# Keyteer/Mixed-precision_LU_Factorization

Measured on AMD Instinct MI355X. Metric: LU GFLOP/s at N=32768 (1/2/4/8 GPUs); IR iterations to ||r||/||b||<1e-12, higher is better.
Workload: dtype f64

## Files before the change

### include/mpf_c.h

```cpp
#ifndef MPF_C_H
#define MPF_C_H
#include <stdint.h>
#ifdef __cplusplus
extern "C" {
#endif

typedef struct mpf_ctx mpf_ctx;

enum { MPF_TRAIL_FP64 = 0, MPF_TRAIL_FP16 = 1, MPF_TRAIL_FP16X3 = 2 };

typedef struct mpf_opts {
    int32_t trailing;
    int32_t verbose;
    int32_t fused_panel;
    int32_t sync_timing;
    int32_t no_lookahead;
    int32_t superpanel;
    int32_t pivot_path;
    int32_t pivot_search;
} mpf_opts;

typedef struct mpf_stats {
    double ms_total;
    double ms_h2d, ms_d2h;
    double ms_hpanel, ms_laswp, ms_dpanel, ms_trsm, ms_gemm;
    int64_t n;
    int32_t nb, panels;
    int32_t hpanel_timeouts;
    int32_t info;
    int32_t gemm_launches;
    int32_t lookahead;
    int32_t superpanel;
    int32_t pivot_path;
    double gemm_flops;
    double gemm_bytes;
    double ms_gemm_big, gemm_big_flops, gemm_big_bytes;
    double ms_cvt;
    double ms_blockrow;
    int32_t gemm_big_launches;
    int32_t host_rows_streamed;
    int32_t host_late_segments;
    int32_t pivot_search;
} mpf_stats;

int mpf_create(mpf_ctx **out, int device);
int mpf_destroy(mpf_ctx *ctx);
int mpf_set_stream(mpf_ctx *ctx, void *hip_stream);
int mpf_synchronize(mpf_ctx *ctx);
const char *mpf_last_error(mpf_ctx *ctx);
int mpf_get_stats(mpf_ctx *ctx, mpf_stats *out);
int64_t mpf_hgetf2_capacity_rows(mpf_ctx *ctx, int32_t waiters, int32_t form);
int mpf_set_option(mpf_ctx *ctx, const char *name, int64_t value);
int mpf_get_option(mpf_ctx *ctx, const char *name, int64_t *value);
int mpf_option_name(int32_t index, char *buf, int64_t buflen);
int mpf_device_report(char *buf, int64_t buflen);


int mpf_factor_host(mpf_ctx *ctx, double *A_host, int64_t N, int32_t nb, int32_t *ipiv_host,
                    const mpf_opts *opts);
int mpf_trim(mpf_ctx *ctx);
int mpf_factor_dev(mpf_ctx *ctx, double *d_A, int64_t lda, int64_t N, int32_t nb, int32_t *d_ipiv,
                   const mpf_opts *opts);

int mpf_double_to_fp16(mpf_ctx *ctx, const double *d_in, uint16_t *d_out, int64_t n);
int mpf_hdiv(mpf_ctx *ctx, const uint16_t *d_a, const uint16_t *d_b, uint16_t *d_q, int64_t n);
int mpf_hgetf2_pivots(mpf_ctx *ctx, const double *d_A, int64_t lda, int32_t rows, int32_t cols,
                      int32_t ipiv_offset, int32_t *d_ipiv, uint16_t *d_panel16_out);
int mpf_hgetf2(mpf_ctx *ctx, uint16_t *d_panel16, int64_t ld, int32_t rows, int32_t cols,
               int32_t *d_ipiv_panel);
int mpf_laswp(mpf_ctx *ctx, double *d_A, int64_t lda, int64_t ncols, int32_t k, int32_t cols,
              const int32_t *d_ipiv_global);
int mpf_dgetf2_npv(mpf_ctx *ctx, double *d_P, int64_t ld, int32_t rows, int32_t cols, int32_t fused);
int mpf_dgetf2_piv(mpf_ctx *ctx, double *d_P, int64_t ld, int32_t rows, int32_t cols, int32_t fused,
                   int32_t ipiv_offset, int32_t *d_ipiv, int32_t *info );
int mpf_dgetf2_tp(mpf_ctx *ctx, double *d_P, int64_t ld, int32_t rows, int32_t cols, int32_t fused,
                  int32_t ipiv_offset, int32_t *d_ipiv, int32_t *info );
int mpf_dtrsm_llnu(mpf_ctx *ctx, int32_t m, int64_t n, const double *d_L, int64_t ldl, double *d_B,
                   int64_t ldb);
int mpf_dgemm_minus(mpf_ctx *ctx, int64_t m, int64_t n, int32_t k, const double *d_A, int64_t lda,
                    const double *d_B, int64_t ldb, double *d_C, int64_t ldc);

int mpf_hgemm_minus(mpf_ctx *ctx, int64_t m, int64_t n, int32_t k, const double *d_A, int64_t lda,
                    const double *d_B, int64_t ldb, double *d_C, int64_t ldc, int32_t split );

int mpf_hgemm_minus_f32(mpf_ctx *ctx, int64_t m, int64_t n, int32_t k, const double *d_A, int64_t lda,
                        const double *d_B, int64_t ldb, float *d_C, int64_t ldc, int32_t split);

int mpf_w32_from_f64(mpf_ctx *ctx, const double *d_A, int64_t lda, float *d_W, int64_t ldw, int64_t rows, int64_t cols);
int mpf_w32_to_f64(mpf_ctx *ctx, const float *d_W, int64_t ldw, double *d_A, int64_t lda, int64_t rows, int64_t cols);
int mpf_w32_laswp(mpf_ctx *ctx, float *d_W, int64_t ldw, int64_t ncols, int32_t k, int32_t cols, const int32_t *d_ipiv_global);

int mpf_matgen_dev(mpf_ctx *ctx, double *d_A, int64_t lda, int64_t N, int64_t skip);
int mpf_matgen_cols_dev(mpf_ctx *ctx, double *d_A, int64_t lda, int64_t N, int64_t skip, int64_t col0, int64_t ncols);
int mpf_matgen_state(int64_t call, uint32_t *out31);

int mpf_check_plu_dev(mpf_ctx *ctx, const double *d_A, int64_t lda, const double *d_LU, int64_t ldlu, const int32_t *d_ipiv,
                      int64_t N, double *max_abs_err, double *fro_rel_err);
int mpf_check_plu_host(const double *A, const double *LU, const int32_t *ipiv, int64_t N, double *max_abs_err, double *fro_rel_err);

typedef struct mpf_ir_stats {
    int32_t iterations;
    int32_t converged;
    double rel_residual;
    double history[32];
    double ms_total;
    int32_t stalled;
    int32_t reserved;
} mpf_ir_stats;
int mpf_solve_ir(mpf_ctx *ctx, const double *d_A, int64_t lda, const double *d_LU, int64_t ldlu,
                 const int32_t *d_ipiv, int64_t N, const double *d_b, double *d_x, int32_t max_iter,
                 double tol, mpf_ir_stats *stats);

int mpf_solve_ir_nrhs(mpf_ctx *ctx, const double *d_A, int64_t lda, const double *d_LU, int64_t ldlu, const int32_t *d_ipiv,
                      int64_t N, int32_t nrhs, const double *d_B, int64_t ldb, double *d_X, int64_t ldx, int32_t max_iter,
                      double tol, mpf_ir_stats *stats);

typedef struct mpf_gmres_stats {
    int32_t outer_iterations, inner_iterations, converged;
    int32_t budget_expired;
    double rel_residual;
    double history[32];
    double ms_total;
} mpf_gmres_stats;
int mpf_solve_gmres_ir(mpf_ctx *ctx, const double *d_A, int64_t lda, const double *d_LU, int64_t ldlu, const int32_t *d_ipiv,
                       int64_t N, const double *d_b, double *d_x, int32_t max_outer, int32_t restart, double tol,
                       mpf_gmres_stats *stats);

typedef struct mpf_gesv_stats {
    int32_t path;
    int32_t info;
    double ms_factor_fp16, ms_ir_fp16, ms_factor_fp64, ms_ir_fp64, ms_total;
    mpf_ir_stats ir_fp16, ir_final;
    double gmres_budget_ms;
    int32_t gmres_budget_expired, reserved;
} mpf_gesv_stats;
int mpf_gesv(mpf_ctx *ctx, const double *d_A, int64_t lda, int64_t N, int32_t nb, double *d_work, int32_t *d_ipiv,
             const double *d_b, double *d_x, int32_t max_iter, double tol,
             int32_t try_fp16 ,
             mpf_gesv_stats *stats);


int mpf_solve_ir_trans(mpf_ctx *ctx, const double *d_A, int64_t lda, const double *d_LU, int64_t ldlu, const int32_t *d_ipiv,
                       int64_t N, int32_t nrhs, const double *d_B, int64_t ldb, double *d_X, int64_t ldx, int32_t max_iter,
                       double tol, mpf_ir_stats *stats);

int mpf_lange(mpf_ctx *ctx, const double *d_A, int64_t lda, int64_t M, int64_t N, char norm, double *out);

int mpf_geequ(mpf_ctx *ctx, const double *d_A, int64_t lda, int64_t N, double *d_r, double *d_c, double *rowcnd, double *colcnd,
              double *amax);

typedef struct mpf_gecon_stats {
    int32_t solves;
    int32_t solves_t;
    int32_t iterations;
    int32_t reserved;
    double ainvnm;
    double ms_total;
} mpf_gecon_stats;
int mpf_gecon(mpf_ctx *ctx, const double *d_LU, int64_t ldlu, int64_t N, char norm, double anorm, double *rcond,
              mpf_gecon_stats *stats);

typedef struct mpf_gesvx_stats {
    int32_t path;
    int32_t info;
    int32_t equed;
    int32_t skipped_by_rcond;
    double rowcnd, colcnd, amax;
    double anorm;
    double kappa_max;
    double rcond_lowp;
    double rcond;
    double ms_equilibrate, ms_factor, ms_gecon, ms_ir, ms_total;
    mpf_ir_stats ir_lowp, ir_final;
} mpf_gesvx_stats;
int mpf_gesvx(mpf_ctx *ctx, const double *d_A, int64_t lda, int64_t N, int32_t nb, double *d_work, int32_t *d_ipiv,
              const double *d_b, double *d_x, int32_t trans, int32_t equilibrate, int32_t try_fp16, double kappa_max,
              int32_t max_iter, double tol, double *d_r, double *d_c, mpf_gesvx_stats *stats);


int mpf_getrs(mpf_ctx *ctx, int32_t trans, const double *d_LU, int64_t ldlu, const int32_t *d_ipiv, int64_t N,
              int32_t nrhs, double *d_B, int64_t ldb);

int mpf_solve_ir_block(mpf_ctx *ctx, int32_t trans, const double *d_A, int64_t lda, const double *d_LU, int64_t ldlu,
                       const int32_t *d_ipiv, int64_t N, int32_t nrhs, const double *d_B, int64_t ldb, double *d_X,
                       int64_t ldx, int32_t max_iter, double tol, mpf_ir_stats *stats);

int mpf_solve_gmres_ir_block(mpf_ctx *ctx, int32_t trans, const double *d_A, int64_t lda, const double *d_LU, int64_t ldlu,
                             const int32_t *d_ipiv, int64_t N, int32_t nrhs, const double *d_B, int64_t ldb, double *d_X, int64_t ldx,
                             int32_t max_outer, int32_t restart, double tol, mpf_gmres_stats *stats );

typedef struct mpf_gerfs_stats {
    int32_t iterations;
    int32_t lacn2_iterations;
    int32_t solves;
    int32_t reserved;
    double ms_total;
} mpf_gerfs_stats;
int mpf_gerfs(mpf_ctx *ctx, int32_t trans, const double *d_A, int64_t lda, const double *d_LU, int64_t ldlu,
              const int32_t *d_ipiv, int64_t N, int32_t nrhs, const double *d_B, int64_t ldb, double *d_X, int64_t ldx,
              int32_t itmax, double *ferr, double *berr, mpf_gerfs_stats *stats);

int mpf_gesvx_block(mpf_ctx *ctx, const double *d_A, int64_t lda, int64_t N, int32_t nb, double *d_work, int32_t *d_ipiv,
                    int32_t nrhs, const double *d_B, int64_t ldb, double *d_X, int64_t ldx,
                    int32_t trans, int32_t equilibrate, int32_t try_fp16, double kappa_max, int32_t max_iter, double tol,
                    int32_t itmax, double *d_r, double *d_c,
                    double *ferr, double *berr,
                    mpf_gesvx_stats *stats,
                    mpf_ir_stats *ir, mpf_gerfs_stats *rfs  );

typedef int (*mpf_bcast_fn)(void *user, void *d_buf, int64_t bytes, int32_t root, void *hip_stream);
typedef int (*mpf_allreduce_fn)(void *user, double *d_buf, int64_t count, void *hip_stream);
typedef struct mpf_dist {
    int32_t rank, world;
    mpf_bcast_fn bcast;
    mpf_allreduce_fn allreduce;
    void *user;
} mpf_dist;
int mpf_rccl_unique_id(void *out128);
int mpf_rccl_init(mpf_ctx *ctx, const void *id128, int32_t rank, int32_t world);
int mpf_rccl_destroy(mpf_ctx *ctx);
int mpf_rccl_version(void);
typedef struct mpf_rccl_info_t {
    int32_t version, has_comm, comm_count, comm_rank, has_p2p, device, visible_devices, reserved;
    int64_t bcast_calls, bcast_bytes, allreduce_calls, p2p_calls, p2p_bytes;
    int32_t link_type[16], link_hops[16], peer_access[16];
} mpf_rccl_info_t;
int mpf_rccl_info(mpf_ctx *ctx, mpf_rccl_info_t *out);
int mpf_rccl_bcast_probe(mpf_ctx *ctx, int64_t bytes, int32_t root, int32_t reps, double *ms_per_bcast);
int mpf_rccl_selftest(mpf_ctx *ctx);
int mpf_factor_dist(mpf_ctx *ctx, double *d_Aloc, int64_t ldloc, int64_t N, int32_t nb, int32_t *d_ipiv, const mpf_dist *dist,
                    const mpf_opts *opts);
typedef int (*mpf_p2p_fn)(void *user, void *d_buf, int64_t bytes, int32_t peer, int32_t send, void *hip_stream);
int mpf_dist_set_p2p(mpf_ctx *ctx, mpf_p2p_fn fn, void *user);
// ... 9 lines not shown
```

### mixed-precision_lu_factorization_amd/__init__.py

```python
import ctypes as C
import os
import subprocess

_HERE = os.path.dirname(os.path.abspath(__file__))
LIB_PATH = os.environ.get("MPF_LIB") or os.path.join(_HERE, "lib", "libmpf_amd.so")
PROBE_LIB_PATH = os.environ.get("MPF_PROBE_LIB") or os.path.join(_HERE, "lib", "libmpf_probe.so")

TRAIL_FP64 = 0
TRAIL_FP16 = 1
TRAIL_FP16X3 = 2

C_ABI_SYMBOLS = [
    "mpf_create", "mpf_destroy", "mpf_set_stream", "mpf_synchronize", "mpf_last_error", "mpf_get_stats",
    "mpf_device_report", "mpf_factor_host", "mpf_factor_dev", "mpf_double_to_fp16", "mpf_hdiv",
    "mpf_hgetf2_pivots", "mpf_hgetf2", "mpf_laswp", "mpf_dgetf2_npv", "mpf_dtrsm_llnu", "mpf_dgemm_minus",
    "mpf_solve_ir", "mpf_hgetf2_capacity_rows", "mpf_set_option", "mpf_get_option", "mpf_option_name", "mpf_hgemm_minus", "mpf_hgemm_minus_f32", "mpf_w32_from_f64", "mpf_w32_to_f64", "mpf_w32_laswp", "mpf_gesv", "mpf_matgen_dev", "mpf_matgen_cols_dev",
    "mpf_matgen_state", "mpf_rccl_unique_id", "mpf_rccl_init", "mpf_rccl_destroy", "mpf_rccl_version", "mpf_rccl_info", "mpf_rccl_bcast_probe", "mpf_factor_dist",
    "mpf_solve_ir_dist", "mpf_rccl_selftest", "mpf_check_plu_dev", "mpf_check_plu_host", "mpf_solve_ir_nrhs",
    "mpf_solve_gmres_ir", "mpf_trim", "mpf_dist_set_p2p",
    "mpf_solve_ir_trans", "mpf_lange", "mpf_geequ", "mpf_gecon", "mpf_gesvx",
    "mpf_getrs", "mpf_solve_ir_block", "mpf_gerfs", "mpf_gesvx_block",
    "mpf_dgetf2_piv", "mpf_solve_gmres_ir_block", "mpf_dgetf2_tp",
]
PROBE_ONLY_SYMBOLS = ["mpf_microbench", "mpf_debug_mfma4", "mpf_debug_gate", "mpf_debug_hgemm_again"]
CXX_SYMBOL_MPF = "_Z3MPFPdiiPi"


class MpfOpts(C.Structure):
    _fields_ = [("trailing", C.c_int32), ("verbose", C.c_int32), ("fused_panel", C.c_int32),
                ("sync_timing", C.c_int32), ("no_lookahead", C.c_int32), ("superpanel", C.c_int32), ("pivot_path", C.c_int32), ("pivot_search", C.c_int32)]


class MpfStats(C.Structure):
    _fields_ = [("ms_total", C.c_double), ("ms_h2d", C.c_double), ("ms_d2h", C.c_double),
                ("ms_hpanel", C.c_double), ("ms_laswp", C.c_double), ("ms_dpanel", C.c_double),
                ("ms_trsm", C.c_double), ("ms_gemm", C.c_double), ("n", C.c_int64), ("nb", C.c_int32),
                ("panels", C.c_int32), ("hpanel_timeouts", C.c_int32), ("info", C.c_int32),
                ("gemm_launches", C.c_int32), ("lookahead", C.c_int32), ("superpanel", C.c_int32),
                ("pivot_path", C.c_int32), ("gemm_flops", C.c_double), ("gemm_bytes", C.c_double),
                ("ms_gemm_big", C.c_double), ("gemm_big_flops", C.c_double), ("gemm_big_bytes", C.c_double),
                ("ms_cvt", C.c_double), ("ms_blockrow", C.c_double), ("gemm_big_launches", C.c_int32), ("host_rows_streamed", C.c_int32),
                ("host_late_segments", C.c_int32), ("pivot_search", C.c_int32)]


class MpfIrStats(C.Structure):
    _fields_ = [("iterations", C.c_int32), ("converged", C.c_int32), ("rel_residual", C.c_double),
                ("history", C.c_double * 32), ("ms_total", C.c_double), ("stalled", C.c_int32), ("reserved", C.c_int32)]


class MpfGmresStats(C.Structure):
    _fields_ = [("outer_iterations", C.c_int32), ("inner_iterations", C.c_int32), ("converged", C.c_int32), ("budget_expired", C.c_int32),
                ("rel_residual", C.c_double), ("history", C.c_double * 32), ("ms_total", C.c_double)]


class MpfRcclInfo(C.Structure):
    _fields_ = [("version", C.c_int32), ("has_comm", C.c_int32), ("comm_count", C.c_int32), ("comm_rank", C.c_int32), ("has_p2p", C.c_int32),
                ("device", C.c_int32), ("visible_devices", C.c_int32), ("reserved", C.c_int32),
                ("bcast_calls", C.c_int64), ("bcast_bytes", C.c_int64), ("allreduce_calls", C.c_int64), ("p2p_calls", C.c_int64), ("p2p_bytes", C.c_int64),
                ("link_type", C.c_int32 * 16), ("link_hops", C.c_int32 * 16), ("peer_access", C.c_int32 * 16)]


class MpfGesvStats(C.Structure):
    _fields_ = [("path", C.c_int32), ("info", C.c_int32), ("ms_factor_fp16", C.c_double), ("ms_ir_fp16", C.c_double),
                ("ms_factor_fp64", C.c_double), ("ms_ir_fp64", C.c_double), ("ms_total", C.c_double),
                ("ir_fp16", MpfIrStats), ("ir_final", MpfIrStats), ("gmres_budget_ms", C.c_double), ("gmres_budget_expired", C.c_int32),
                ("reserved", C.c_int32)]


class MpfGeconStats(C.Structure):
    _fields_ = [("solves", C.c_int32), ("solves_t", C.c_int32), ("iterations", C.c_int32), ("reserved", C.c_int32),
                ("ainvnm", C.c_double), ("ms_total", C.c_double)]


class MpfGesvxStats(C.Structure):
    _fields_ = [("path", C.c_int32), ("info", C.c_int32), ("equed", C.c_int32), ("skipped_by_rcond", C.c_int32),
                ("rowcnd", C.c_double), ("colcnd", C.c_double), ("amax", C.c_double), ("anorm", C.c_double), ("kappa_max", C.c_double),
                ("rcond_lowp", C.c_double), ("rcond", C.c_double), ("ms_equilibrate", C.c_double), ("ms_factor", C.c_double),
                ("ms_gecon", C.c_double), ("ms_ir", C.c_double), ("ms_total", C.c_double), ("ir_lowp", MpfIrStats), ("ir_final", MpfIrStats)]


class MpfGerfsStats(C.Structure):
    _fields_ = [("iterations", C.c_int32), ("lacn2_iterations", C.c_int32), ("solves", C.c_int32), ("reserved", C.c_int32),
                ("ms_total", C.c_double)]


BCAST_FN = C.CFUNCTYPE(C.c_int, C.c_void_p, C.c_void_p, C.c_int64, C.c_int32, C.c_void_p)
ALLREDUCE_FN = C.CFUNCTYPE(C.c_int, C.c_void_p, C.c_void_p, C.c_int64, C.c_void_p)
P2P_FN = C.CFUNCTYPE(C.c_int, C.c_void_p, C.c_void_p, C.c_int64, C.c_int32, C.c_int32, C.c_void_p)


class MpfDist(C.Structure):
    _fields_ = [("rank", C.c_int32), ("world", C.c_int32), ("bcast", BCAST_FN), ("allreduce", ALLREDUCE_FN), ("user", C.c_void_p)]


class MPFError(RuntimeError):
    pass


def build(force=False):
    srcs = [os.path.join(_HERE, "csrc", f) for f in os.listdir(os.path.join(_HERE, "csrc"))]
    srcs += [os.path.join(_HERE, "..", "include", h) for h in ("mpf_c.h", "MPF.h", "mpf_probe.h")] + [os.path.join(_HERE, "Makefile")]
    stale = force or any(not os.path.exists(lp) or any(os.path.getmtime(s) > os.path.getmtime(lp) for s in srcs)
                         for lp in (LIB_PATH, PROBE_LIB_PATH))
    if stale:
        subprocess.run(["make", "-C", _HERE, "-s", "-j8", "all", "probe"], check=True)
    return LIB_PATH


_libs = {}


def load_library(probe=False):
    if probe in _libs:
        return _libs[probe]
    import torch
    path = PROBE_LIB_PATH if probe else LIB_PATH
    if not os.path.exists(path):
        raise MPFError(f"{path} is missing: run `python -c 'import __graft_entry__ as g; g.build()'` "
                       "(there is no CPU fallback)")
    L = C.CDLL(path)
    vp, i32, i64, dbl = C.c_void_p, C.c_int32, C.c_int64, C.c_double
    L.mpf_create.argtypes = [C.POINTER(vp), C.c_int]
    L.mpf_destroy.argtypes = [vp]
    L.mpf_set_stream.argtypes = [vp, vp]
    L.mpf_synchronize.argtypes = [vp]
    L.mpf_last_error.argtypes = [vp]
    L.mpf_last_error.restype = C.c_char_p
    L.mpf_get_stats.argtypes = [vp, C.POINTER(MpfStats)]
    L.mpf_set_option.argtypes = [vp, C.c_char_p, i64]
    L.mpf_get_option.argtypes = [vp, C.c_char_p, C.POINTER(i64)]
    L.mpf_option_name.argtypes = [i32, C.c_char_p, i64]
    L.mpf_device_report.argtypes = [C.c_char_p, i64]
    L.mpf_factor_host.argtypes = [vp, vp, i64, i32, vp, C.POINTER(MpfOpts)]
    L.mpf_trim.argtypes = [vp]
    L.mpf_dist_set_p2p.argtypes = [vp, P2P_FN, vp]
    L.mpf_factor_dev.argtypes = [vp, vp, i64, i64, i32, vp, C.POINTER(MpfOpts)]
    L.mpf_double_to_fp16.argtypes = [vp, vp, vp, i64]
    L.mpf_hdiv.argtypes = [vp, vp, vp, vp, i64]
    L.mpf_hgetf2_pivots.argtypes = [vp, vp, i64, i32, i32, i32, vp, vp]
    L.mpf_hgetf2.argtypes = [vp, vp, i64, i32, i32, vp]
    L.mpf_laswp.argtypes = [vp, vp, i64, i64, i32, i32, vp]
    L.mpf_dgetf2_npv.argtypes = [vp, vp, i64, i32, i32, i32]
    L.mpf_dgetf2_piv.argtypes = [vp, vp, i64, i32, i32, i32, i32, vp, C.POINTER(i32)]
    L.mpf_dgetf2_tp.argtypes = [vp, vp, i64, i32, i32, i32, i32, vp, C.POINTER(i32)]
    L.mpf_dtrsm_llnu.argtypes = [vp, i32, i64, vp, i64, vp, i64]
    L.mpf_dgemm_minus.argtypes = [vp, i64, i64, i32, vp, i64, vp, i64, vp, i64]
    L.mpf_hgemm_minus.argtypes = [vp, i64, i64, i32, vp, i64, vp, i64, vp, i64, i32]
    L.mpf_hgemm_minus_f32.argtypes = [vp, i64, i64, i32, vp, i64, vp, i64, vp, i64, i32]
    L.mpf_w32_from_f64.argtypes = [vp, vp, i64, vp, i64, i64, i64]
    L.mpf_w32_to_f64.argtypes = [vp, vp, i64, vp, i64, i64, i64]
    L.mpf_w32_laswp.argtypes = [vp, vp, i64, i64, i32, i32, vp]
    L.mpf_solve_ir.argtypes = [vp, vp, i64, vp, i64, vp, i64, vp, vp, i32, dbl, C.POINTER(MpfIrStats)]
    L.mpf_solve_ir_nrhs.argtypes = [vp, vp, i64, vp, i64, vp, i64, i32, vp, i64, vp, i64, i32, dbl, C.POINTER(MpfIrStats)]
    L.mpf_solve_gmres_ir.argtypes = [vp, vp, i64, vp, i64, vp, i64, vp, vp, i32, i32, dbl, C.POINTER(MpfGmresStats)]
    L.mpf_gesv.argtypes = [vp, vp, i64, i64, i32, vp, vp, vp, vp, i32, dbl, i32, C.POINTER(MpfGesvStats)]
    L.mpf_solve_ir_trans.argtypes = [vp, vp, i64, vp, i64, vp, i64, i32, vp, i64, vp, i64, i32, dbl, C.POINTER(MpfIrStats)]
    L.mpf_lange.argtypes = [vp, vp, i64, i64, i64, C.c_char, C.POINTER(dbl)]
    L.mpf_geequ.argtypes = [vp, vp, i64, i64, vp, vp, C.POINTER(dbl), C.POINTER(dbl), C.POINTER(dbl)]
    L.mpf_gecon.argtypes = [vp, vp, i64, i64, C.c_char, dbl, C.POINTER(dbl), C.POINTER(MpfGeconStats)]
    L.mpf_gesvx.argtypes = [vp, vp, i64, i64, i32, vp, vp, vp, vp, i32, i32, i32, dbl, i32, dbl, vp, vp, C.POINTER(MpfGesvxStats)]
    L.mpf_getrs.argtypes = [vp, i32, vp, i64, vp, i64, i32, vp, i64]
    L.mpf_solve_ir_block.argtypes = [vp, i32, vp, i64, vp, i64, vp, i64, i32, vp, i64, vp, i64, i32, dbl, C.POINTER(MpfIrStats)]
    L.mpf_solve_gmres_ir_block.argtypes = [vp, i32, vp, i64, vp, i64, vp, i64, i32, vp, i64, vp, i64, i32, i32, dbl, C.POINTER(MpfGmresStats)]
    L.mpf_gerfs.argtypes = [vp, i32, vp, i64, vp, i64, vp, i64, i32, vp, i64, vp, i64, i32, C.POINTER(dbl), C.POINTER(dbl),
                            C.POINTER(MpfGerfsStats)]
    L.mpf_gesvx_block.argtypes = [vp, vp, i64, i64, i32, vp, vp, i32, vp, i64, vp, i64, i32, i32, i32, dbl, i32, dbl, i32, vp, vp,
                                  C.POINTER(dbl), C.POINTER(dbl), C.POINTER(MpfGesvxStats), C.POINTER(MpfIrStats), C.POINTER(MpfGerfsStats)]
    L.mpf_matgen_dev.argtypes = [vp, vp, i64, i64, i64]
    L.mpf_matgen_cols_dev.argtypes = [vp, vp, i64, i64, i64, i64, i64]
    L.mpf_matgen_state.argtypes = [i64, C.POINTER(C.c_uint32)]
    L.mpf_rccl_unique_id.argtypes = [vp]
    L.mpf_rccl_init.argtypes = [vp, vp, i32, i32]
    L.mpf_rccl_destroy.argtypes = [vp]
    L.mpf_rccl_version.argtypes = []
    L.mpf_rccl_selftest.argtypes = [vp]
    L.mpf_check_plu_dev.argtypes = [vp, vp, i64, vp, i64, vp, i64, C.POINTER(dbl), C.POINTER(dbl)]
    L.mpf_check_plu_host.argtypes = [vp, vp, vp, i64, C.POINTER(dbl), C.POINTER(dbl)]
    L.mpf_factor_dist.argtypes = [vp, vp, i64, i64, i32, vp, C.POINTER(MpfDist), C.POINTER(MpfOpts)]
    L.mpf_solve_ir_dist.argtypes = [vp, vp, i64, vp, i64, vp, i64, i32, vp, vp, i32, dbl, C.POINTER(MpfDist), C.POINTER(MpfIrStats)]
    for name in C_ABI_SYMBOLS:
        if name != "mpf_last_error":
            getattr(L, name).restype = C.c_int
    if probe:
        L.mpf_microbench.argtypes = [vp, C.c_int, C.POINTER(C.c_double)]
        L.mpf_microbench.restype = C.c_int
    _libs[probe] = L
    return L


def option_names():
    L = load_library()
    buf = C.create_string_buffer(64)
    n = L.mpf_option_name(-1, buf, 64)
    out = []
    for i in range(n):
        L.mpf_option_name(i, buf, 64)
        out.append(buf.value.decode())
    return out


def device_report():
    L = load_library()
    buf = C.create_string_buffer(4096)
    n = L.mpf_device_report(buf, 4096)
    return n, buf.value.decode()


def _ptr(t):
    return C.c_void_p(t.data_ptr()) if t is not None else C.c_void_p(0)


def _colmajor_ld(t):
    assert t.dim() == 2 and t.stride(0) == 1, "need a column-major matrix (e.g. X.t() of a contiguous tensor)"
    return t.stride(1) if t.shape[1] > 1 else max(t.shape[0], 1)


class MPFContext:

    def __init__(self, device=0, use_torch_stream=True, stream=None, probe=False, options=None):
        import torch
        if not torch.cuda.is_available():
            raise MPFError("no GPU visible: the MPF hot path is HIP-only (no CPU fallback)")
        self.torch = torch
        self.probe = probe
        self.L = load_library(probe)
        self.h = C.c_void_p()
        rc = self.L.mpf_create(C.byref(self.h), device)
        if rc != 0:
            raise MPFError("mpf_create failed: " + self.L.mpf_last_error(None).decode())
        self.device = torch.device("cuda", device)
        self.stream = stream
        self._follow = stream is None and use_torch_stream
        self._bound = None
        if stream is not None:
            self.L.mpf_set_stream(self.h, C.c_void_p(stream.cuda_stream))
        self._bind()
        for k, v in (options or {}).items():
            self.set_option(k, v)

    def set_option(self, name, value):
        self._check(self.L.mpf_set_option(self.h, name.encode(), int(value)), "mpf_set_option")

    def rccl_info(self):
        inf = MpfRcclInfo()
        self.L.mpf_rccl_info.argtypes = [C.c_void_p, C.POINTER(MpfRcclInfo)]
        self._check(self.L.mpf_rccl_info(self.h, C.byref(inf)), "mpf_rccl_info")
        nd = min(int(inf.visible_devices), 16)
        return {"version": int(inf.version), "has_comm": bool(inf.has_comm), "comm_count": int(inf.comm_count), "comm_rank": int(inf.comm_rank),
                "has_p2p": bool(inf.has_p2p), "device": int(inf.device), "visible_devices": int(inf.visible_devices),
                "bcast_calls": int(inf.bcast_calls), "bcast_bytes": int(inf.bcast_bytes), "allreduce_calls": int(inf.allreduce_calls),
                "p2p_calls": int(inf.p2p_calls), "p2p_bytes": int(inf.p2p_bytes),
                "link_type_to_device": [int(inf.link_type[d]) for d in range(nd)], "link_hops_to_device": [int(inf.link_hops[d]) for d in range(nd)],
                "peer_access_to_device": [int(inf.peer_access[d]) for d in range(nd)]}

    def rccl_bcast_probe(self, nbytes, root=0, reps=5):
        self._bind()
        ms = C.c_double(0)
        self.L.mpf_rccl_bcast_probe.argtypes = [C.c_void_p, C.c_int64, C.c_int32, C.c_int32, C.POINTER(C.c_double)]
        self._check(self.L.mpf_rccl_bcast_probe(self.h, int(nbytes), int(root), int(reps), C.byref(ms)), "mpf_rccl_bcast_probe")
        return ms.value

    def hgetf2_capacity_rows(self, waiters=0, form=0):
        self.L.mpf_hgetf2_capacity_rows.argtypes = [C.c_void_p, C.c_int32, C.c_int32]
        self.L.mpf_hgetf2_capacity_rows.restype = C.c_int64
        return int(self.L.mpf_hgetf2_capacity_rows(self.h, waiters, form))

    def get_option(self, name):
        v = C.c_int64(0)
        self._check(self.L.mpf_get_option(self.h, name.encode(), C.byref(v)), "mpf_get_option")
        return v.value

    def _bind(self):
        if self._follow:
            cur = self.torch.cuda.current_stream(self.device).cuda_stream
            if cur != self._bound:
                self.L.mpf_set_stream(self.h, C.c_void_p(cur))
                self._bound = cur

    def close(self):
        if self.h:
            self.L.mpf_destroy(self.h)
            self.h = C.c_void_p()

    def __del__(self):
        try:
            self.close()
        except Exception:
            pass

    def _check(self, rc, what):
        if rc < 0:
            raise MPFError(f"{what} failed ({rc}): " + self.L.mpf_last_error(self.h).decode())
        return rc

    def colmajor(self, rows, cols, dtype=None):
        t = self.torch
        return t.empty((cols, rows), dtype=dtype or t.float64, device=self.device).t()

    def from_numpy_f(self, a):
# ... 79 lines not shown
        n, nrhs = B.shape
        X = self.colmajor(n, nrhs)
        st = (MpfIrStats * nrhs)()
        rc = self.L.mpf_solve_ir_nrhs(self.h, _ptr(A), _colmajor_ld(A), _ptr(LU), _colmajor_ld(LU), _ptr(ipiv), n, nrhs,
                                      _ptr(B), _colmajor_ld(B), _ptr(X), _colmajor_ld(X), max_iter, tol, st)
        self._check(rc, "mpf_solve_ir_nrhs")
        return X, list(st)

    def solve_gmres_ir(self, A, LU, ipiv, b, max_outer=10, restart=30, tol=1e-12):
        self._bind()
        t = self.torch
        n = A.shape[0]
        x = t.empty(n, dtype=t.float64, device=self.device)
        st = MpfGmresStats()
        rc = self.L.mpf_solve_gmres_ir(self.h, _ptr(A), _colmajor_ld(A), _ptr(LU), _colmajor_ld(LU), _ptr(ipiv), n, _ptr(b), _ptr(x),
                                       max_outer, restart, tol, C.byref(st))
        self._check(rc, "mpf_solve_gmres_ir")
        return x, st

    def check_plu(self, A, LU, ipiv):
        self._bind()
        mx, fro = C.c_double(0), C.c_double(0)
        rc = self.L.mpf_check_plu_dev(self.h, _ptr(A), _colmajor_ld(A), _ptr(LU), _colmajor_ld(LU), _ptr(ipiv), A.shape[0],
                                      C.byref(mx), C.byref(fro))
        self._check(rc, "mpf_check_plu_dev")
        return mx.value, fro.value

    def rccl_init(self, rank, world, group=None):
        import torch.distributed as tdist
        ident = [None]
        if world == 1:
            buf = C.create_string_buffer(128)
            self._check(self.L.mpf_rccl_unique_id(buf), "mpf_rccl_unique_id")
            self._check(self.L.mpf_rccl_init(self.h, buf, 0, 1), "mpf_rccl_init")
            return
        loaded = [int(self.L.mpf_rccl_version() > 0)]
        everyone = [None] * world
        tdist.all_gather_object(everyone, loaded[0], group=group)
        if not all(everyone):
            raise RuntimeError(f"librccl not loadable on ranks {[r for r, ok in enumerate(everyone) if not ok]}")
        if rank == 0:
            buf = C.create_string_buffer(128)
            if self.L.mpf_rccl_unique_id(buf) == 0:
                ident[0] = bytes(buf.raw)
        tdist.broadcast_object_list(ident, src=0, group=group)
        if ident[0] is None:
            raise RuntimeError("mpf_rccl_unique_id failed on rank 0 (librccl not loadable?)")
        self._check(self.L.mpf_rccl_init(self.h, C.c_char_p(ident[0]), rank, world), "mpf_rccl_init")

    def dist_set_p2p(self, fn):
        self._bind()
        self._check(self.L.mpf_dist_set_p2p(self.h, fn if fn is not None else C.cast(None, P2P_FN), None), "mpf_dist_set_p2p")

    def factor_dist(self, Aloc, n, nb, dist, ipiv=None, trailing=TRAIL_FP64, no_lookahead=False, pivot_path=0, verbose=False, superpanel=0,
                    pivot_search=0):
        self._bind()
        t = self.torch
        if ipiv is None:
            ipiv = t.arange(1, n + 1, dtype=t.int32, device=self.device)
        o = MpfOpts(trailing=trailing, no_lookahead=int(no_lookahead), pivot_path=int(pivot_path), verbose=int(verbose), superpanel=int(superpanel),
                    pivot_search=int(pivot_search))
        ld = _colmajor_ld(Aloc) if Aloc.shape[1] > 0 else n
        rc = self.L.mpf_factor_dist(self.h, _ptr(Aloc) if Aloc.shape[1] > 0 else C.c_void_p(0), max(ld, n), n, nb, _ptr(ipiv),
                                    C.byref(dist), C.byref(o))
        return ipiv, self._check(rc, "mpf_factor_dist")

    def solve_ir_dist(self, Aloc, LUloc, ipiv, b, n, nb, dist, max_iter=10, tol=1e-12):
        self._bind()
        t = self.torch
        x = t.empty(n, dtype=t.float64, device=self.device)
        st = MpfIrStats()
        has = Aloc.shape[1] > 0
        rc = self.L.mpf_solve_ir_dist(self.h, _ptr(Aloc) if has else C.c_void_p(0), max(_colmajor_ld(Aloc), n) if has else n,
                                      _ptr(LUloc) if has else C.c_void_p(0), max(_colmajor_ld(LUloc), n) if has else n, _ptr(ipiv),
                                      n, nb, _ptr(b), _ptr(x), max_iter, tol, C.byref(dist), C.byref(st))
        self._check(rc, "mpf_solve_ir_dist")
        return x, st

    def double_to_fp16(self, x):
        self._bind()
        t = self.torch
        out = t.empty(x.numel(), dtype=t.int16, device=self.device)
        self._check(self.L.mpf_double_to_fp16(self.h, _ptr(x), _ptr(out), x.numel()), "double_to_fp16")
        return out

    def hdiv(self, a_bits, b_bits):
        self._bind()
        t = self.torch
        q = t.empty_like(a_bits)
        self._check(self.L.mpf_hdiv(self.h, _ptr(a_bits), _ptr(b_bits), _ptr(q), a_bits.numel()), "hdiv")
        return q

    def hgetf2_pivots(self, P, ipiv_offset=0, want_panel=False):
        self._bind()
        t = self.torch
        rows, cols = P.shape
        ipiv = t.zeros(cols, dtype=t.int32, device=self.device)
        out = self.colmajor(rows, cols, dtype=t.int16) if want_panel else None
        rc = self.L.mpf_hgetf2_pivots(self.h, _ptr(P), _colmajor_ld(P), rows, cols, ipiv_offset, _ptr(ipiv), _ptr(out))
        self._check(rc, "hgetf2_pivots")
        return ipiv, out

    def hgetf2(self, P16):
        self._bind()
        t = self.torch
        rows, cols = P16.shape
        ipiv = t.zeros(cols, dtype=t.int32, device=self.device)
        self._check(self.L.mpf_hgetf2(self.h, _ptr(P16), _colmajor_ld(P16), rows, cols, _ptr(ipiv)), "hgetf2")
        return ipiv

    def laswp(self, A, k, cols, ipiv_global):
        self._bind()
        self._check(self.L.mpf_laswp(self.h, _ptr(A), _colmajor_ld(A), A.shape[1], k, cols, _ptr(ipiv_global)), "laswp")

    def dgetf2_npv(self, P, fused=False):
        self._bind()
        rows, cols = P.shape
        self._check(self.L.mpf_dgetf2_npv(self.h, _ptr(P), _colmajor_ld(P), rows, cols, int(fused)), "dgetf2_npv")

    def dgetf2_piv(self, P, fused=False, ipiv_offset=0):
        self._bind()
        t = self.torch
        rows, cols = P.shape
        ipiv = t.zeros(min(rows, cols), dtype=t.int32, device=self.device)
        info = C.c_int32(0)
        self._check(self.L.mpf_dgetf2_piv(self.h, _ptr(P), _colmajor_ld(P), rows, cols, int(fused), int(ipiv_offset), _ptr(ipiv),
                                          C.byref(info)), "dgetf2_piv")
        return ipiv, info.value

    def dgetf2_tp(self, P, fused=False, ipiv_offset=0):
        self._bind()
        t = self.torch
        rows, cols = P.shape
        ipiv = t.zeros(min(rows, cols), dtype=t.int32, device=self.device)
        info = C.c_int32(0)
        self._check(self.L.mpf_dgetf2_tp(self.h, _ptr(P), _colmajor_ld(P), rows, cols, int(fused), int(ipiv_offset), _ptr(ipiv),
                                         C.byref(info)), "dgetf2_tp")
        return ipiv, info.value

    def dtrsm_llnu(self, Lm, B):
        self._bind()
        m, n = B.shape
        assert Lm.shape[0] >= m and Lm.shape[1] >= m, "dtrsm_llnu: L smaller than m x m"
        self._check(self.L.mpf_dtrsm_llnu(self.h, m, n, _ptr(Lm), _colmajor_ld(Lm), _ptr(B), _colmajor_ld(B)), "dtrsm")

    def dgemm_minus(self, Cm, A, B):
        self._bind()
        m, n = Cm.shape
        k = A.shape[1]
        assert A.shape == (m, k) and B.shape == (k, n), "dgemm_minus: operand shapes do not match C"
        self._check(self.L.mpf_dgemm_minus(self.h, m, n, k, _ptr(A), _colmajor_ld(A), _ptr(B), _colmajor_ld(B),
                                           _ptr(Cm), _colmajor_ld(Cm)), "dgemm")

    def hgemm_minus(self, Cm, A, B, split=False):
        self._bind()
        m, n = Cm.shape
        k = A.shape[1]
        assert A.shape == (m, k) and B.shape == (k, n), "hgemm_minus: operand shapes do not match C"
        self._check(self.L.mpf_hgemm_minus(self.h, m, n, k, _ptr(A), _colmajor_ld(A), _ptr(B), _colmajor_ld(B),
                                           _ptr(Cm), _colmajor_ld(Cm), int(split)), "hgemm")

    def hgemm_minus_f32(self, Cm, A, B, split=False):
        self._bind()
        assert Cm.dtype == self.torch.float32
        m, n = Cm.shape
        k = A.shape[1]
        assert A.shape == (m, k) and B.shape == (k, n), "hgemm_minus_f32: operand shapes do not match C"
        self._check(self.L.mpf_hgemm_minus_f32(self.h, m, n, k, _ptr(A), _colmajor_ld(A), _ptr(B), _colmajor_ld(B),
                                               _ptr(Cm), _colmajor_ld(Cm), int(split)), "hgemm_f32")

    def w32_from_f64(self, A, W):
        self._bind()
        rows, cols = A.shape
        assert W.shape == (rows, cols) and W.dtype == self.torch.float32 and W.stride(1) == 1
        self._check(self.L.mpf_w32_from_f64(self.h, _ptr(A), _colmajor_ld(A), _ptr(W), W.stride(0), rows, cols), "w32_from_f64")

    def w32_to_f64(self, W, A):
        self._bind()
        rows, cols = A.shape
        assert W.shape == (rows, cols) and W.dtype == self.torch.float32 and W.stride(1) == 1
        self._check(self.L.mpf_w32_to_f64(self.h, _ptr(W), W.stride(0), _ptr(A), _colmajor_ld(A), rows, cols), "w32_to_f64")

    def w32_laswp(self, W, k, cols, ipiv_global):
        self._bind()
        assert W.dtype == self.torch.float32 and W.stride(1) == 1
        self._check(self.L.mpf_w32_laswp(self.h, _ptr(W), W.stride(0), W.shape[1], k, cols, _ptr(ipiv_global)), "w32_laswp")

    def gesv(self, A, b, nb=256, max_iter=10, tol=1e-12, try_fp16=True, work=None):
        self._bind()
        t = self.torch
        n = A.shape[0]
        if work is None:
            work = self.colmajor(n, n)
        ipiv = t.empty(n, dtype=t.int32, device=self.device)
        x = t.empty(n, dtype=t.float64, device=self.device)
        st = MpfGesvStats()
        rc = self.L.mpf_gesv(self.h, _ptr(A), _colmajor_ld(A), n, nb, _ptr(work), _ptr(ipiv), _ptr(b), _ptr(x), max_iter, tol,
                             int(try_fp16), C.byref(st))
        self._check(rc, "mpf_gesv")
        return x, st, work, ipiv

    def solve_ir_trans(self, A, LU, ipiv, B, max_iter=10, tol=1e-12):
        self._bind()
        n = A.shape[0]
        vec = B.dim() == 1
        nrhs = 1 if vec else B.shape[1]
        X = self.torch.empty(n, dtype=self.torch.float64, device=self.device) if vec else self.colmajor(n, nrhs)
        st = (MpfIrStats * max(nrhs, 1))()
        ldb = n if vec else _colmajor_ld(B)
        ldx = n if vec else _colmajor_ld(X)
        rc = self.L.mpf_solve_ir_trans(self.h, _ptr(A), _colmajor_ld(A), _ptr(LU), _colmajor_ld(LU), _ptr(ipiv), n, nrhs,
                                       _ptr(B), ldb, _ptr(X), ldx, max_iter, tol, st)
        self._check(rc, "mpf_solve_ir_trans")
        return X, (st[0] if vec else list(st)[:nrhs])

    def lange(self, A, norm="1"):
        self._bind()
        m, n = A.shape
        out = C.c_double(0)
        ld = _colmajor_ld(A) if m > 0 and n > 0 else max(m, 1)
        self._check(self.L.mpf_lange(self.h, _ptr(A), ld, m, n, norm.encode()[:1], C.byref(out)), "mpf_lange")
        return out.value

    def geequ(self, A):
        self._bind()
        t = self.torch
        n = A.shape[0]
        r = t.zeros(n, dtype=t.float64, device=self.device)
        c = t.zeros(n, dtype=t.float64, device=self.device)
        rc_, cc_, am = C.c_double(0), C.c_double(0), C.c_double(0)
        info = self._check(self.L.mpf_geequ(self.h, _ptr(A), _colmajor_ld(A), n, _ptr(r), _ptr(c), C.byref(rc_), C.byref(cc_), C.byref(am)),
                           "mpf_geequ")
        return r, c, rc_.value, cc_.value, am.value, info

    def gecon(self, LU, anorm, norm="1"):
        self._bind()
        rcond = C.c_double(0)
        st = MpfGeconStats()
        self._check(self.L.mpf_gecon(self.h, _ptr(LU), _colmajor_ld(LU), LU.shape[0], norm.encode()[:1], float(anorm), C.byref(rcond),
                                     C.byref(st)), "mpf_gecon")
        return rcond.value, st

    def cond(self, A, LU, ipiv=None, norm="1"):
        anorm = self.lange(A, norm)
        rcond, _ = self.gecon(LU, anorm, norm)
        return float("inf") if rcond == 0 else 1.0 / rcond

    def gesvx(self, A, b, nb=256, trans=False, equilibrate=1, try_fp16=1, kappa_max=0.0, max_iter=10, tol=1e-12, work=None,
              want_scales=False):
        self._bind()
        t = self.torch
        n = A.shape[0]
        if work is None:
            work = self.colmajor(n, n)
        ipiv = t.empty(n, dtype=t.int32, device=self.device)
        x = t.empty(n, dtype=t.float64, device=self.device)
        r = t.empty(n, dtype=t.float64, device=self.device) if want_scales else None
        c = t.empty(n, dtype=t.float64, device=self.device) if want_scales else None
        st = MpfGesvxStats()
        rc = self.L.mpf_gesvx(self.h, _ptr(A), _colmajor_ld(A), n, nb, _ptr(work), _ptr(ipiv), _ptr(b), _ptr(x), int(bool(trans)),
                              int(equilibrate), int(try_fp16), float(kappa_max), max_iter, tol, _ptr(r), _ptr(c), C.byref(st))
        self._check(rc, "mpf_gesvx")
        out = (x, st, work, ipiv)
        return out + (r, c) if want_scales else out

    def _rhs(self, B):
        if B.dim() == 1:
            return B.view(-1, 1), 1, max(B.shape[0], 1)
        return B, B.shape[1], _colmajor_ld(B)

    def getrs(self, LU, ipiv, B, trans=False, overwrite=False):
        self._bind()
        n = LU.shape[0]
        if overwrite:
            X = B
        elif B.dim() == 1:
            X = B.clone()
        else:
            X = self.colmajor(n, B.shape[1])
            X.copy_(B)
        _, nrhs, ldx = self._rhs(X)
        rc = self.L.mpf_getrs(self.h, int(bool(trans)), _ptr(LU), _colmajor_ld(LU), _ptr(ipiv), n, nrhs, _ptr(X), ldx)
        self._check(rc, "mpf_getrs")
        return X

    def solve_ir_block(self, A, LU, ipiv, B, trans=False, max_iter=10, tol=1e-12):
        self._bind()
        n = A.shape[0]
        vec = B.dim() == 1
        _, nrhs, ldb = self._rhs(B)
        X = self.torch.empty(n, dtype=self.torch.float64, device=self.device) if vec else self.colmajor(n, nrhs)
        ldx = n if vec else _colmajor_ld(X)
        st = (MpfIrStats * max(nrhs, 1))()
        rc = self.L.mpf_solve_ir_block(self.h, int(bool(trans)), _ptr(A), _colmajor_ld(A), _ptr(LU), _colmajor_ld(LU), _ptr(ipiv), n,
                                       nrhs, _ptr(B), ldb, _ptr(X), ldx, max_iter, tol, st)
        self._check(rc, "mpf_solve_ir_block")
        return X, list(st)[:nrhs]

    def solve_gmres_ir_block(self, A, LU, ipiv, B, trans=False, max_outer=10, restart=30, tol=1e-12):
        self._bind()
        n = A.shape[0]
        vec = B.dim() == 1
        _, nrhs, ldb = self._rhs(B)
        X = self.torch.empty(n, dtype=self.torch.float64, device=self.device) if vec else self.colmajor(n, nrhs)
        ldx = n if vec else _colmajor_ld(X)
        st = (MpfGmresStats * max(nrhs, 1))()
# ... 57 lines not shown
```

### mixed-precision_lu_factorization_amd/csrc/mpf_host.cpp

```cpp
#include "solve_common.h"
#include "../../include/MPF.h"
#include <climits>
#include <cstdio>
#include <cstdlib>
#include <cstring>
#include <cmath>
#include <iostream>
#include <vector>
#include <mutex>
#include <functional>
#include <chrono>

static thread_local std::string g_noctx_err;

namespace {
struct OptDesc { const char *name, *env; size_t off; bool wide; long long lo, hi; };
#define OPT_I(field, env, lo, hi) {#field, env, offsetof(MpfTuning, field), false, lo, hi}
#define OPT_L(field, env, lo, hi) {#field, env, offsetof(MpfTuning, field), true, lo, hi}
const OptDesc kOpts[] = {
    OPT_I(safe_pivots, "MPF_SAFE_PIVOTS", 0, 1),
    OPT_I(pivot_fp64, "MPF_PIVOT_FP64", 0, 2),
    OPT_I(chain_pipeline, "MPF_CHAIN_PIPELINE", 0, 1),
    OPT_L(chain_pipeline_below, "MPF_CHAIN_PIPELINE_BELOW", 0, 1ll << 40),
    OPT_I(fp16_work32, "MPF_FP16_WORK32", 0, 1),
    OPT_I(superpanel_fp16, "MPF_SUPERPANEL", 0, 8),
    OPT_I(superpanel_fp64, "MPF_SUPERPANEL_FP64", 1, 8),
    OPT_I(no_lookahead, "MPF_NO_LOOKAHEAD", 0, 1),
    OPT_I(verbose, "MPF_VERBOSE", 0, 1),
    OPT_I(timeline, "MPF_TIMELINE", 0, 1),
    OPT_L(hp_spin_limit, "MPF_HP_SPIN_LIMIT", 1, 1ll << 31),
    OPT_L(hp_gate_ticks, "MPF_HP_GATE_TICKS", 0, 1ll << 40),
    OPT_I(hp_acq_fence, "MPF_HP_ACQ_FENCE", 0, 1),
    OPT_I(hp_window, "MPF_HP_WINDOW", -1, 1 << 30),
    OPT_I(hgemm_pad, "MPF_HGEMM_PAD", 0, 65536),
    OPT_I(hgemm_split_pad, "MPF_HGEMM_SPLIT_PAD", 0, 65536),
    OPT_I(hgemm_big, "MPF_HGEMM_BIG", 0, 1),
    OPT_I(hgemm_big_tile, "MPF_HGEMM_BIG_TILE", 0, 5),
    OPT_I(hgemm_mfma16, "MPF_HGEMM_MFMA16", 0, 1),
    OPT_I(dgemm_dma, "MPF_DGEMM_DMA", 0, 1),
    OPT_I(lazy_gather, "MPF_LAZY_GATHER", 0, 1),
    OPT_I(dpanel_fused_form, "MPF_DPANEL_FUSED", 0, 1),
    OPT_I(dist_instalments, "MPF_DIST_INSTALMENTS", 0, 1),
    OPT_L(dist_instalment_min_bytes, "MPF_DIST_INSTALMENT_MIN_BYTES", 0, 1ll << 40),
    OPT_I(generic_fused, "MPF_GENERIC_FUSED", 0, 1),
    OPT_I(fp64_rowmajor, "MPF_FP64_ROWMAJOR", 0, 1),
    OPT_L(fp64_rowmajor_min_n, "MPF_FP64_ROWMAJOR_MIN_N", 0, 1ll << 40),
    OPT_I(trsm_laswp_fused, "MPF_TRSM_LASWP_FUSED", 0, 1),
    OPT_I(fp64_two_lanes, "MPF_FP64_TWO_LANES", 0, 1 << 30),
    OPT_I(fp64_lane_a_pct, "MPF_FP64_LANE_A_PCT", 20, 90),
    OPT_I(fp64_pair, "MPF_FP64_PAIR", 0, 1),
    OPT_L(fp64_pair_min_n, "MPF_FP64_PAIR_MIN_N", 0, 1ll << 40),
    OPT_I(event_timers, "MPF_EVENT_TIMERS", 0, 2),
    OPT_I(dist_world1_loop, "MPF_DIST_WORLD1_LOOP", 0, 1),
    OPT_I(gesv_fp64_tflops, "MPF_GESV_FP64_TFLOPS", 0, 1000),
    OPT_I(gate_wait_value, "MPF_GATE_WAIT_VALUE", 0, 1),
    OPT_I(host_sink, "MPF_HOST_SINK", 0, 1),
    OPT_I(sink_trace, "MPF_SINK_TRACE", 0, 1),
    OPT_I(hp_half_slabs, "MPF_HP_HALF_SLABS", 0, 1),
    OPT_I(hp_half_slabs_rows, "MPF_HP_HALF_SLABS_ROWS", 256, 32768),
    OPT_I(hp_local_xcd, "MPF_HP_LOCAL_XCD", 0, 2),
    OPT_I(host_late_parts, "MPF_HOST_LATE_PARTS", 0, 4),
    OPT_L(host_late_min_n, "MPF_HOST_LATE_MIN_N", 0, 1ll << 40),
    OPT_I(host_first_pct, "MPF_HOST_FIRST_PCT", 5, 100),
    OPT_I(host_late_q_pct, "MPF_HOST_LATE_Q_PCT", 1, 1000),
    OPT_L(host_sink_min_n, "MPF_HOST_SINK_MIN_N", 0, 1ll << 40),
    OPT_I(dist_solve_p2p, "MPF_DIST_SOLVE_P2P", 0, 1),
    OPT_I(gmres_group_tiles, "MPF_GMRES_GROUP_TILES", 0, 16),
#ifdef MPF_PROBE
    OPT_I(hp_stamp, "MPF_HP_STAMP", 0, 1),
    OPT_I(hp_r256_upto, "MPF_HP_R256_UPTO", 0, 1 << 30),
    OPT_I(dgemm_w8, "MPF_DGEMM_W8", 0, 1),
    OPT_I(gemm_lds_pad, "MPF_GEMM_LDS_PAD", 0, 65536),
    OPT_I(hgemm_big_reg, "MPF_HGEMM_BIG_REG", 0, 1),
    OPT_I(hgemm_dbg, "MPF_HGEMM_DBG", 0, 8191),
#endif
};
#undef OPT_I
#undef OPT_L
void opt_store(MpfTuning &t, const OptDesc &d, long long v) {
    if (v < d.lo) v = d.lo;
    if (v > d.hi) v = d.hi;
    char *p = (char *)&t + d.off;
    if (d.wide) *(long long *)p = v; else *(int *)p = (int)v;
}
long long opt_load(const MpfTuning &t, const OptDesc &d) {
    const char *p = (const char *)&t + d.off;
    return d.wide ? *(const long long *)p : (long long)*(const int *)p;
}
void tuning_from_env(MpfTuning &t) {
    for (const OptDesc &d : kOpts)
        if (const char *e = getenv(d.env)) if (*e) opt_store(t, d, atoll(e));
}
}

static int fail(mpf_ctx *c, int code, const std::string &msg) {
    if (c) c->err = msg; else g_noctx_err = msg;
    return code;
}

extern "C" {

int mpf_create(mpf_ctx **out, int device) {
    if (!out) return -1;
    *out = nullptr;
    int ndev = 0;
    hipError_t e = hipGetDeviceCount(&ndev);
    if (e != hipSuccess || ndev == 0) return fail(nullptr, -3, "No HIP devices available.");
    if (device < 0 || device >= ndev) return fail(nullptr, -1, "mpf_create: bad device index");
    mpf_ctx *c = new mpf_ctx();
    tuning_from_env(c->tune);
    c->device = device;
    if (hipSetDevice(device) != hipSuccess) { delete c; return fail(nullptr, -2, "hipSetDevice failed"); }
    hipDeviceProp_t prop;
    if (hipGetDeviceProperties(&prop, device) == hipSuccess) c->num_cus = prop.multiProcessorCount;
    if (hipStreamCreateWithFlags(&c->stream, hipStreamNonBlocking) != hipSuccess) { delete c; return fail(nullptr, -2, "hipStreamCreate failed"); }
    c->own_stream = true;
    {
        int lo = 0, hi = 0;
        hipDeviceGetStreamPriorityRange(&lo, &hi);
        if (hipStreamCreateWithPriority(&c->pstream, hipStreamNonBlocking, hi) != hipSuccess) c->pstream = nullptr;
        if (hipStreamCreateWithPriority(&c->tstream, hipStreamNonBlocking, hi) != hipSuccess) c->tstream = nullptr;
    }
    if (hipMalloc((void **)&c->ws, sizeof(MpfWorkspace)) != hipSuccess) { hipStreamDestroy(c->stream); delete c; return fail(nullptr, -2, "hipMalloc(workspace) failed"); }
    hipMemset(c->ws, 0, sizeof(MpfWorkspace));
    if (hipExtMallocWithFlags((void **)&c->hp_signal, 8, hipMallocSignalMemory) != hipSuccess) { c->hp_signal = nullptr; (void)hipGetLastError(); }
    else hipMemset(c->hp_signal, 0, 8);
    hipEventCreate(&c->ev0);
    hipEventCreate(&c->ev1);
    *out = c;
    return 0;
}

int mpf_destroy(mpf_ctx *c) {
    if (!c) return 0;
    hipSetDevice(c->device);
    if (c->stream) hipStreamSynchronize(c->stream);
    if (c->ws) hipFree(c->ws);
    if (c->hp_signal) hipFree(c->hp_signal);
    mpf_rccl_destroy(c);
    sink_destroy(c);
    feed_destroy(c);
    if (c->ev0) hipEventDestroy(c->ev0);
    if (c->ev1) hipEventDestroy(c->ev1);
    if (c->pstream) { hipStreamSynchronize(c->pstream); hipStreamDestroy(c->pstream); }
    if (c->tstream) { hipStreamSynchronize(c->tstream); hipStreamDestroy(c->tstream); }
    if (c->xstream) { hipStreamSynchronize(c->xstream); hipStreamDestroy(c->xstream); }
    for (hipEvent_t e : c->ev_pool) hipEventDestroy(e);
    if (c->own_stream && c->stream) hipStreamDestroy(c->stream);
    delete c;
    return 0;
}

int mpf_set_stream(mpf_ctx *c, void *hip_stream) {
    if (!c) return -1;
    if (c->own_stream && c->stream) { hipStreamSynchronize(c->stream); hipStreamDestroy(c->stream); }
    c->stream = (hipStream_t)hip_stream;
    c->own_stream = false;
    return 0;
}

int mpf_synchronize(mpf_ctx *c) {
    if (!c) return -1;
    MPF_HIP_TRY(c, hipStreamSynchronize(c->stream));
    return 0;
}

const char *mpf_last_error(mpf_ctx *c) { return c ? c->err.c_str() : g_noctx_err.c_str(); }

int mpf_get_stats(mpf_ctx *c, mpf_stats *out) {
    if (!c || !out) return -1;
    *out = c->stats;
    return 0;
}

int mpf_set_option(mpf_ctx *c, const char *name, int64_t value) {
    if (!c || !name) return -1;
    for (const OptDesc &d : kOpts)
        if (!strcmp(d.name, name)) {
            opt_store(c->tune, d, (long long)value);
            c->attr_done = 0; c->attr_big = 0;
            return 0;
        }
    return fail(c, -1, std::string("mpf_set_option: unknown option '") + name + "'");
}
int mpf_get_option(mpf_ctx *c, const char *name, int64_t *value) {
    if (!c || !name || !value) return -1;
    for (const OptDesc &d : kOpts)
        if (!strcmp(d.name, name)) { *value = (int64_t)opt_load(c->tune, d); return 0; }
    return fail(c, -1, std::string("mpf_get_option: unknown option '") + name + "'");
}
int mpf_option_name(int32_t index, char *buf, int64_t buflen) {
    const int n = (int)(sizeof kOpts / sizeof kOpts[0]);
    if (index >= 0 && index < n && buf && buflen > 0) { strncpy(buf, kOpts[index].name, (size_t)buflen - 1); buf[buflen - 1] = 0; }
    return n;
}

int mpf_device_report(char *buf, int64_t buflen) {
    int ndev = 0;
    if (hipGetDeviceCount(&ndev) != hipSuccess) ndev = 0;
    std::string s = "HIP devices: " + std::to_string(ndev) + "\n";
    int rt = 0, drv = 0;
    if (ndev > 0 && hipRuntimeGetVersion(&rt) == hipSuccess && hipDriverGetVersion(&drv) == hipSuccess)
        s += "HIP runtime " + std::to_string(rt) + " driver " + std::to_string(drv) + "\n";
    const int rv = ndev > 0 ? mpf_rccl_version() : -1;
    s += rv > 0 ? "RCCL version " + std::to_string(rv / 10000) + "." + std::to_string(rv / 100 % 100) + "." + std::to_string(rv % 100) + " (NCCL API, dlopen)\n"
                : std::string("RCCL: not loaded\n");
    for (int d = 0; d < ndev; ++d) {
        hipDeviceProp_t p;
        if (hipGetDeviceProperties(&p, d) != hipSuccess) continue;
        int coop = 0, lds_cu = 0, l2 = 0, clk = 0, memclk = 0, buswidth = 0;
        hipDeviceGetAttribute(&coop, hipDeviceAttributeCooperativeLaunch, d);
        hipDeviceGetAttribute(&lds_cu, hipDeviceAttributeMaxSharedMemoryPerMultiprocessor, d);
        hipDeviceGetAttribute(&l2, hipDeviceAttributeL2CacheSize, d);
        hipDeviceGetAttribute(&clk, hipDeviceAttributeClockRate, d);
        hipDeviceGetAttribute(&memclk, hipDeviceAttributeMemoryClockRate, d);
        hipDeviceGetAttribute(&buswidth, hipDeviceAttributeMemoryBusWidth, d);
        char line[768];
        snprintf(line, sizeof line,
                 "device %d: %s arch %s CUs %d maxThreadsPerBlock %d LDS/block %zu B LDS/CU %d B warpSize %d regs/block %d "
                 "L2 %d KiB clock %d MHz memclock %d MHz bus %d bit HBM %.1f GiB cooperativeLaunch %d pivot-kernel rows/launch %d\n",
                 d, p.name, p.gcnArchName, p.multiProcessorCount, p.maxThreadsPerBlock, p.sharedMemPerBlock, lds_cu, p.warpSize,
                 p.regsPerBlock, l2 / 1024, clk / 1000, memclk / 1000, buswidth, (double)p.totalGlobalMem / (1024.0 * 1024.0 * 1024.0), coop,
                 HP_R * (p.multiProcessorCount < HP_MAXG ? p.multiProcessorCount : HP_MAXG));
        s += line;
    }
    if (ndev > 1) {
        s += "link matrix (type:hops, type 4 = xGMI; P = peer access):\n";
        for (int a = 0; a < ndev; ++a) {
            std::string row = "  dev " + std::to_string(a) + ":";
            for (int b = 0; b < ndev; ++b) {
                if (a == b) { row += "   -  "; continue; }
                uint32_t lt = 0, hops = 0;
                int peer = 0;
                hipDeviceCanAccessPeer(&peer, a, b);
                if (hipExtGetLinkTypeAndHopCount(a, b, &lt, &hops) != hipSuccess) { lt = 0; hops = 0; }
                char cell[32];
                snprintf(cell, sizeof cell, " %u:%u%s", lt, hops, peer ? "P" : " ");
                row += cell;
            }
            s += row + "\n";
        }
    }
    if (buf && buflen > 0) { strncpy(buf, s.c_str(), (size_t)buflen - 1); buf[buflen - 1] = 0; }
    return ndev;
}

int mpf_double_to_fp16(mpf_ctx *c, const double *d_in, uint16_t *d_out, int64_t n) {
    if (!c) return -1;
    return launch_double_to_fp16(c, d_in, d_out, n);
}
int mpf_hdiv(mpf_ctx *c, const uint16_t *a, const uint16_t *b, uint16_t *q, int64_t n) {
    if (!c) return -1;
    return launch_hdiv(c, a, b, q, n);
}
int mpf_hgetf2_pivots(mpf_ctx *c, const double *d_A, int64_t lda, int32_t rows, int32_t cols, int32_t ipiv_offset,
                      int32_t *d_ipiv, uint16_t *d_panel16_out) {
    if (!c || !d_A || !d_ipiv) return -1;
    if (lda < rows) return fail(c, -1, "hgetf2_pivots: lda < rows");
    if (cols > 65535) return fail(c, -1, "hgetf2_pivots: panel width > 65535");
    if (!safe_pivots(c) && hgetf2_lds_eligible(c, rows, cols))
        return launch_hgetf2(c, d_A, lda, nullptr, 0, rows, cols, ipiv_offset, d_ipiv, d_panel16_out, rows, nullptr);
    return launch_hgetf2_generic(c, d_A, lda, nullptr, 0, rows, cols, ipiv_offset, d_ipiv, d_panel16_out, rows);
}
int mpf_hgetf2(mpf_ctx *c, uint16_t *d_panel16, int64_t ld, int32_t rows, int32_t cols, int32_t *d_ipiv_panel) {
    if (!c || !d_panel16 || !d_ipiv_panel) return -1;
    if (ld < rows) return fail(c, -1, "hgetf2: ld < rows");
    if (!safe_pivots(c) && hgetf2_lds_eligible(c, rows, cols))
        return launch_hgetf2(c, nullptr, 0, d_panel16, ld, rows, cols, 0, d_ipiv_panel, nullptr, 0, nullptr);
    return launch_hgetf2_generic(c, nullptr, 0, d_panel16, ld, rows, cols, 0, d_ipiv_panel, nullptr, 0);
}
int mpf_laswp(mpf_ctx *c, double *d_A, int64_t lda, int64_t ncols, int32_t k, int32_t cols, const int32_t *d_ipiv) {
    if (!c || !d_A || !d_ipiv) return -1;
    if (cols > HP_MAXCOLS) return launch_laswp_seq(c, d_A, lda, ncols, k, cols, d_ipiv, lda);
    return launch_laswp(c, d_A, lda, ncols, k, cols, d_ipiv);
}
int mpf_dgetf2_npv(mpf_ctx *c, double *d_P, int64_t ld, int32_t rows, int32_t cols, int32_t fused) {
    if (!c || !d_P) return -1;
    if (ld < rows) return fail(c, -1, "dgetf2_npv: ld < rows");
    return launch_dgetf2_npv(c, d_P, ld, rows, cols, fused, 0);
}
int mpf_dgetf2_piv(mpf_ctx *c, double *d_P, int64_t ld, int32_t rows, int32_t cols, int32_t fused, int32_t ipiv_offset,
                   int32_t *d_ipiv, int32_t *info) {
    if (!c || !d_P || !d_ipiv) return -1;
    if (rows < 1 || cols < 1 || cols > 65535) return fail(c, -1, "dgetf2_piv: need rows >= 1 and 1 <= cols <= 65535");
    if (ld < rows) return fail(c, -1, "dgetf2_piv: ld < rows");
    MPF_HIP_TRY(c, hipSetDevice(c->device));
    const int imax = INT_MAX;
    MPF_HIP_TRY(c, hipMemcpyAsync(&c->ws->info, &imax, sizeof(int), hipMemcpyHostToDevice, c->stream));
    const int rc = launch_dgetf2_piv(c, d_P, ld, rows, cols, fused, 0, ipiv_offset, d_ipiv);
    if (rc || !info) return rc;
    int v = 0;
    MPF_HIP_TRY(c, hipMemcpyAsync(&v, &c->ws->info, sizeof(int), hipMemcpyDeviceToHost, c->stream));
    MPF_HIP_TRY(c, hipStreamSynchronize(c->stream));
    *info = v == INT_MAX ? 0 : v;
    return 0;
}
int mpf_dgetf2_tp(mpf_ctx *c, double *d_P, int64_t ld, int32_t rows, int32_t cols, int32_t fused, int32_t ipiv_offset,
                  int32_t *d_ipiv, int32_t *info) {
    if (!c || !d_P || !d_ipiv) return -1;
    if (rows < 1 || cols < 1 || cols > 65535) return fail(c, -1, "dgetf2_tp: need rows >= 1 and 1 <= cols <= 65535");
    if (ld < rows) return fail(c, -1, "dgetf2_tp: ld < rows");
    MPF_HIP_TRY(c, hipSetDevice(c->device));
    const int imax = INT_MAX;
    MPF_HIP_TRY(c, hipMemcpyAsync(&c->ws->info, &imax, sizeof(int), hipMemcpyHostToDevice, c->stream));
    const int rc = launch_dgetf2_tp(c, d_P, ld, rows, cols, fused, 0, ipiv_offset, d_ipiv);
    if (rc || !info) return rc;
    int v = 0;
    MPF_HIP_TRY(c, hipMemcpyAsync(&v, &c->ws->info, sizeof(int), hipMemcpyDeviceToHost, c->stream));
    MPF_HIP_TRY(c, hipStreamSynchronize(c->stream));
    *info = v == INT_MAX ? 0 : v;
    return 0;
}
int mpf_dtrsm_llnu(mpf_ctx *c, int32_t m, int64_t n, const double *d_L, int64_t ldl, double *d_B, int64_t ldb) {
    if (!c) return -1;
    if (m > 0 && n > 0 && (ldl < m || ldb < m)) return fail(c, -1, "dtrsm: leading dimension < m");
    return launch_dtrsm_llnu(c, m, n, d_L, ldl, d_B, ldb);
}
int mpf_dgemm_minus(mpf_ctx *c, int64_t m, int64_t n, int32_t k, const double *d_A, int64_t lda, const double *d_B,
                    int64_t ldb, double *d_C, int64_t ldc) {
    if (!c) return -1;
    if (m > 0 && n > 0 && k > 0 && (lda < m || ldb < k || ldc < m)) return fail(c, -1, "dgemm: bad leading dimension");
    return launch_dgemm_minus(c, m, n, k, d_A, lda, d_B, ldb, d_C, ldc);
}

int mpf_ensure_h_images(mpf_ctx *c, int64_t rows, int kmax, bool big) {
    kmax = (kmax + 63) & ~63;
    if (c->h_L && c->h_rows >= rows && c->h_kmax >= kmax && (!big || c->h_Lb[0])) return 0;
    if (rows < c->h_rows) rows = c->h_rows;
    if (kmax < c->h_kmax) kmax = c->h_kmax;
    big = big || c->h_Lb[0];
    c->h_L.release(); c->h_U.release();
    for (auto &b : c->h_Lb) b.release();
    c->h_rows = 0; c->h_kmax = 0;
    const int64_t elems = 2 * rows * kmax;
    MPF_HIP_TRY(c, c->h_L.grow(elems));
    MPF_HIP_TRY(c, c->h_U.grow(elems));
    if (big) for (auto &b : c->h_Lb) MPF_HIP_TRY(c, b.grow(elems));
    c->h_rows = rows; c->h_kmax = kmax;
    return 0;
}

int mpf_hgemm_minus(mpf_ctx *c, int64_t m, int64_t n, int32_t k, const double *d_A, int64_t lda, const double *d_B,
                    int64_t ldb, double *d_C, int64_t ldc, int32_t split) {
    if (!c) return -1;
    if (m <= 0 || n <= 0 || k <= 0) return 0;
    if (k > 8 * HP_MAXCOLS) return fail(c, -1, "hgemm: k > 2048");
    if (lda < m || ldb < k || ldc < m) return fail(c, -1, "hgemm: bad leading dimension");
    int rc = mpf_ensure_h_images(c, m > n ? m : n, k, false);
    if (!rc) rc = launch_cvt_l21(c, d_A, lda, m, k, split);
    if (!rc) rc = launch_hgemm_minus(c, m, n, k, d_B, ldb, d_C, ldc, split);
    return rc;
}

int mpf_hgemm_minus_f32(mpf_ctx *c, int64_t m, int64_t n, int32_t k, const double *d_A, int64_t lda, const double *d_B,
                        int64_t ldb, float *d_C, int64_t ldc, int32_t split) {
    if (!c || !d_A || !d_B || !d_C) return -1;
    if (m <= 0 || n <= 0 || k <= 0) return 0;
    if (k > 8 * HP_MAXCOLS) return fail(c, -1, "hgemm: k > 2048");
    if (lda < m || ldb < k || ldc < m) return fail(c, -1, "hgemm: bad leading dimension");
    int rc = mpf_ensure_h_images(c, m > n ? m : n, k, false);
    if (!rc) rc = launch_cvt_l21(c, d_A, lda, m, k, split);
    c->hgemm_standalone = true;
    if (!rc) rc = launch_hgemm_minus_w32(c, m, n, k, d_B, ldb, d_C, ldc, split);
    c->hgemm_standalone = false;
    return rc;
}

int mpf_w32_from_f64(mpf_ctx *c, const double *d_A, int64_t lda, float *d_W, int64_t ldw, int64_t rows, int64_t cols) {
    if (!c || !d_A || !d_W) return -1;
    if (lda < rows || ldw < cols) return fail(c, -1, "w32_from_f64: bad leading dimension");
    return launch_cvt_f64_f32(c, d_A, lda, d_W, ldw, rows, cols);
}
int mpf_w32_to_f64(mpf_ctx *c, const float *d_W, int64_t ldw, double *d_A, int64_t lda, int64_t rows, int64_t cols) {
    if (!c || !d_A || !d_W) return -1;
    if (lda < rows || ldw < cols) return fail(c, -1, "w32_to_f64: bad leading dimension");
    return launch_cvt_f32_f64(c, d_W, ldw, d_A, lda, rows, cols);
}
int mpf_w32_laswp(mpf_ctx *c, float *d_W, int64_t ldw, int64_t ncols, int32_t k, int32_t cols, const int32_t *d_ipiv) {
    if (!c || !d_W || !d_ipiv) return -1;
    if (cols < 1 || cols > HP_MAXCOLS) return fail(c, -1, "w32_laswp: 1 <= cols <= 256");
    if (ldw < ncols) return fail(c, -1, "w32_laswp: ldw < ncols");
    const int64_t need = (int64_t)LASWP_MAXMOVED * ncols / 2 + 1;
    if (need > c->perm_tmp.cap()) {
        MPF_HIP_TRY(c, hipStreamSynchronize(c->stream));
        MPF_HIP_TRY(c, c->perm_tmp.grow(need));
    }
    int rc = launch_laswp_plan(c, d_ipiv, k, cols, &c->ws->list0);
    if (!rc) rc = launch_laswp_from_list_f32(c, d_W, ldw, ncols, &c->ws->list0);
    return rc;
}


static int trail_gemm(mpf_ctx *c, const mpf_opts &o, int64_t m, int64_t n, int pc, const double *L21, const double *U12,
                      double *C, int64_t lda) {
    if (o.trailing != MPF_TRAIL_FP64) return launch_hgemm_minus(c, m, n, pc, U12, lda, C, lda, o.trailing == MPF_TRAIL_FP16X3);
    return launch_dgemm_minus(c, m, n, pc, L21, lda, U12, lda, C, lda);
}

struct FactorArgs {
    mpf_ctx *c; EvPool &ev; mpf_stats &st; const mpf_opts &o;
    double *d_A; int64_t lda, N; int32_t nb; int32_t *d_ipiv;
};

static int pref_window_rows(const mpf_opts &o) { return o.trailing == MPF_TRAIL_FP64 ? HP_FP64_WINDOW_ROWS : 0; }

static void stream_join(EvPool &ev, hipStream_t from, hipStream_t into) {
    hipEvent_t e = ev.get();
    hipEventRecord(e, from);
    hipStreamWaitEvent(into, e, 0);
}

static int factor_sync_timed(mpf_ctx *c, double *d_A, int64_t lda, int64_t N, int32_t nb, int32_t *d_ipiv,
                             const mpf_opts &o, mpf_stats &st) {
    hipEvent_t pe0, pe1;
    hipEventCreate(&pe0); hipEventCreate(&pe1);
    auto phase = [&](double &acc, auto &&fn) -> int {
        hipEventRecord(pe0, c->stream);
        int rc = fn();
        hipEventRecord(pe1, c->stream);
        hipEventSynchronize(pe1);
        float ms = 0; hipEventElapsedTime(&ms, pe0, pe1);
        acc += ms;
        return rc;
    };
    int rc = 0;
    for (int64_t k = 0; k < N && rc == 0; k += nb) {
        const int pc = (int)((N - k) < nb ? (N - k) : nb);
        const int pr = (int)(N - k);
        if (pr <= 1) break;
        double *Ap = d_A + k * lda + k;
        MovedList *ml = c->lists + (k / nb);
        rc = phase(st.ms_hpanel, [&] { return launch_hgetf2(c, Ap, lda, nullptr, 0, pr, pc, (int)k, d_ipiv + k, nullptr, 0, ml, 0, pref_window_rows(o)); });
        if (rc) break;
        rc = phase(st.ms_laswp, [&] { return launch_laswp_from_list(c, d_A + k * lda, lda, N - k, ml); });
        if (rc) break;
        rc = phase(st.ms_dpanel, [&] { return launch_dgetf2_npv(c, Ap, lda, pr, pc, o.fused_panel, (int)k); });
        if (rc) break;
        if (k + pc < N) {
            const int64_t n = N - k - pc;
            double *A12 = d_A + (k + pc) * lda + k;
            rc = phase(st.ms_trsm, [&] { return launch_dtrsm_llnu(c, pc, n, Ap, lda, A12, lda); });
            if (rc) break;
            rc = phase(st.ms_gemm, [&] {
                int e = o.trailing != MPF_TRAIL_FP64 ? launch_cvt_l21(c, Ap + pc, lda, n, pc, o.trailing == MPF_TRAIL_FP16X3) : 0;
                if (!e) e = trail_gemm(c, o, n, n, pc, Ap + pc, A12, A12 + pc, lda);
                return e; });
            if (rc) break;
            count_gemm(st, o, n, n, pc);
        }
        st.panels++;
        if (o.verbose) printf("panel k=%lld rows=%d cols=%d\n", (long long)k, pr, pc);
    }
    if (!rc) rc = phase(st.ms_laswp, [&] { return launch_lazy_left_swaps(c, d_A, lda, N, nb, (int)((N + nb - 1) / nb), c->lists); });
    hipEventDestroy(pe0); hipEventDestroy(pe1);
    return rc;
}

static int factor_generic(mpf_ctx *c, double *d_A, int64_t lda, int64_t N, int32_t nb, int32_t *d_ipiv, const mpf_opts &o,
                          mpf_stats &st, bool force_generic_pivots, int piv64) {
    EvPool ev(c);
    ev.keep = &st.ms_gemm;
    hipStream_t S = c->stream;
    int rc = 0;
    const bool split = o.trailing == MPF_TRAIL_FP16X3;
    for (int64_t k = 0; k < N && rc == 0; k += nb) {
        const int pc = (int)((N - k) < nb ? (N - k) : nb);
        const int pr = (int)(N - k);
        if (pr <= 1) break;
        double *Ap = d_A + k * lda + k;
        if (piv64) {
            rc = ev.timed(st.ms_dpanel, S, [&] {
                return piv64 == 2 ? launch_dgetf2_tp(c, Ap, lda, pr, pc, o.fused_panel, (int)k, (int)k, d_ipiv + k)
                                  : launch_dgetf2_piv(c, Ap, lda, pr, pc, o.fused_panel, (int)k, (int)k, d_ipiv + k); });
            if (rc) break;
            rc = ev.timed(st.ms_laswp, S, [&] {
// ... 382 lines not shown
            rc = ev.timed(st.ms_hpanel, P, [&] {
                int e = launch_hgetf2(c, d_A, lda, nullptr, 0, (int)N, pc0, 0, d_ipiv, nullptr, 0, c->lists, 0, pref_window_rows(o));
                if (!e) e = launch_laswp_from_list(c, d_A, lda, pc0, c->lists);
                if (!e) e = launch_dgetf2_npv(c, d_A, lda, (int)N, pc0, o.fused_panel, 0);
                return e; });
            hipEventRecord(e0, P);
        }
        st.panels++;
        if (!rc && pc0 < ce) rc = ev.timed(st.ms_cvt, S, [&] { return launch_transpose64(c, d_A + (int64_t)pc0 * lda, lda, R + pc0, ldr, N, ce - pc0, true); });
        hipStreamWaitEvent(S, e0, 0);
        chain_a = e0;
    }
    int64_t cm = -1;
    hipEvent_t doneL = nullptr, doneR = nullptr, prevR = nullptr;
    hipEvent_t init_done = ev.get();
    hipEventRecord(init_done, S);
    bool was_two = false;
    int64_t k0 = 0;
    if (pairs && !rc && !sink && !lp && T && N > 1) {
        PairHandover h;
        h.chain = chain_a;
        rc = factor_rm_pairs(c, ev, st, o, d_A, lda, N, nb, d_ipiv, init_done, h);
        if (h.k0 > 0) {
            k0 = h.k0; chain_a = h.chain; doneL = h.doneL; doneR = h.doneR; cm = h.cm;
            was_two = true;
        }
    }
    for (int64_t k = k0; k < N && rc == 0; k += nb) {
        const int pc = (int)((N - k) < nb ? (N - k) : nb);
        if (N - k <= 1 || k + pc >= N) break;
        const int64_t n = N - k - pc;
        const int64_t nx = k + pc;
        const int pc2 = (int)((N - nx) < nb ? (N - nx) : nb);
        const bool has_next = (N - nx) > 1;
        double *Ap = d_A + k * lda + k;
        double *LT = c->rm_lt + ((k / nb) & 1) * N * (int64_t)nb;
        const int64_t ns = has_next ? pc2 : n;
        MovedList *lk = c->lists + (k / nb);
        while (lp && lseg < lp->nseg && (k / nb >= lp->q[lseg] || nx + pc2 > ce || !has_next)) {
            const int64_t c_lo = lp->c0[lseg], c_hi = lseg + 1 < lp->nseg ? lp->c0[lseg + 1] : N, w = c_hi - c_lo;
            double *LT3 = c->rm_lt + 2 * N * (int64_t)nb;
            rc = launch_late_wait(c, lp->flags + lseg, lp->seq);
            if (!rc && lp->snapshot) {
                MPF_HIP_TRY(c, hipMemcpyAsync(lp->snapshot + c_lo * N, d_A + c_lo * lda, (size_t)w * N * sizeof(double), hipMemcpyDeviceToDevice, S));
                lp->snapped[lseg] = true;
            }
            if (!rc) rc = ev.timed(st.ms_cvt, S, [&] { return launch_transpose64(c, d_A + c_lo * lda, lda, R + c_lo, ldr, N, w, true); });
            for (int64_t kj = 0; kj < k && rc == 0; kj += nb) {
                const int64_t nxj = kj + nb, nj = N - nxj;
                double *Apj = d_A + kj * lda + kj;
                const MovedList *lj = c->lists + (kj / nb);
                rc = ev.timed(st.ms_cvt, S, [&] { return launch_transpose64(c, Apj + nb, lda, LT3, nb, nj, nb, true); });
                if (!rc) rc = ev.timed(st.ms_laswp, S, [&] { return launch_laswp_from_list_rm64(c, R + c_lo, ldr, w, lj, (int64_t)LASWP_MAXMOVED * c_lo); });
                if (!rc) rc = ev.timed(st.ms_trsm, S, [&] { return launch_dtrsm_llnu_strided(c, nb, w, Apj, lda, R + kj * ldr + c_lo, ldr, 1); });
                if (!rc) rc = ev.timed(st.ms_cvt, S, [&] { return launch_transpose64(c, d_A + c_lo * lda + kj, lda, R + kj * ldr + c_lo, ldr, nb, w, false); });
                if (!rc) rc = ev.timed(st.ms_gemm, S, [&] { return launch_dgemm_minus(c, w, nj, nb, R + kj * ldr + c_lo, ldr, LT3, nb, R + nxj * ldr + c_lo, ldr); });
                count_gemm(st, o, nj, w, nb);
                if (sink && !rc && c_hi == N) sink_notify(c, (int)(kj / nb) + 1, S);
            }
            ++lseg;
            ce = lseg < lp->nseg ? lp->c0[lseg] : N;
            cm = -1;
            doneR = ev.get();
            hipEventRecord(doneR, S);
            doneL = nullptr;
        }
        if (rc) break;
        const int64_t cw = ce - nx - pc2;
        const bool want_two = T && c->tune.fp64_two_lanes > 0 && has_next && pivots_fit_beside_update(c, N - nx) &&
                              (N - nx) > c->tune.chain_pipeline_below && cw >= c->tune.fp64_two_lanes;
        if (!want_two) cm = -1;
        const bool resplit = want_two && lane_split(c, nx + pc2, ce, cm);
        if (cm >= 0) {
            const int64_t aw = cm - (nx + pc2);
            if (!was_two && k > 0) {
                doneL = ev.get();
                hipEventRecord(doneL, S);
            }
            hipEvent_t lt_ready = ev.get();
            {
                if (prevR) hipStreamWaitEvent(P, prevR, 0);
                StreamSwap sw(c, P);
                rc = ev.timed(st.ms_cvt, P, [&] { return launch_transpose64(c, Ap + pc, lda, LT, pc, n, pc, true); });
                hipEventRecord(lt_ready, P);
            }
            if (rc) break;
            hipEvent_t e1 = ev.get(), e2 = ev.get(), evA = ev.get(), evB = ev.get();
            {
                if (chain_a) hipStreamWaitEvent(T, chain_a, 0);
                if (chain_b) hipStreamWaitEvent(T, chain_b, 0);
                if (doneL) hipStreamWaitEvent(T, doneL, 0); else hipStreamWaitEvent(T, init_done, 0);
                if (resplit && doneR) hipStreamWaitEvent(T, doneR, 0);
                StreamSwap sw(c, T);
                rc = ev.timed(st.ms_laswp, T, [&] { return launch_laswp_from_list_rm64(c, R + nx, ldr, cm - nx, lk); });
                if (!rc) rc = ev.timed(st.ms_trsm, T, [&] { return launch_dtrsm_llnu_strided(c, pc, ns, Ap, lda, R + k * ldr + nx, ldr, 1); });
                hipStreamWaitEvent(T, lt_ready, 0);
                if (!rc) rc = ev.timed(st.ms_gemm, T, [&] { return launch_dgemm_minus(c, ns, n, pc, R + k * ldr + nx, ldr, LT, pc, R + nx * ldr + nx, ldr); });
                count_gemm(st, o, n, ns, pc);
                if (!rc) rc = ev.timed(st.ms_cvt, T, [&] { return launch_transpose64(c, d_A + nx * lda + nx, lda, R + nx * ldr + nx, ldr, N - nx, pc2, false); });
                hipEventRecord(e1, T);
            }
            if (rc) break;
            {
                hipStreamWaitEvent(P, e1, 0);
                if (doneR) hipStreamWaitEvent(P, doneR, 0);
                rc = panel_chain(f, nx, P);
                hipEventRecord(e2, P);
            }
            if (rc) break;
            {
                StreamSwap sw(c, T);
                rc = ev.timed(st.ms_trsm, T, [&] { return launch_dtrsm_llnu_strided(c, pc, aw, Ap, lda, R + k * ldr + nx + pc2, ldr, 1); });
                if (!rc) rc = ev.timed(st.ms_cvt, T, [&] { return launch_transpose64(c, d_A + nx * lda + k, lda, R + k * ldr + nx, ldr, pc, cm - nx, false); });
                hipEventRecord(evA, T);
                if (doneR) hipStreamWaitEvent(T, doneR, 0);
                if (!rc) rc = ev.timed(st.ms_laswp, T, [&] { return launch_laswp_from_list_rm64(c, R + cm, ldr, ce - cm, lk, (int64_t)LASWP_MAXMOVED * (cm - nx)); });
                if (!rc) rc = ev.timed(st.ms_trsm, T, [&] { return launch_dtrsm_llnu_strided(c, pc, ce - cm, Ap, lda, R + k * ldr + cm, ldr, 1); });
                if (!rc) rc = ev.timed(st.ms_cvt, T, [&] { return launch_transpose64(c, d_A + cm * lda + k, lda, R + k * ldr + cm, ldr, pc, ce - cm, false); });
                hipEventRecord(evB, T);
                if (sink && !rc && ce == N) sink_notify(c, (int)(k / nb) + 1, T);
            }
            if (rc) break;
            hipStreamWaitEvent(S, evA, 0);
            rc = ev.timed(st.ms_gemm, S, [&] { return launch_dgemm_minus(c, aw, n, pc, R + k * ldr + nx + pc2, ldr, LT, pc, R + nx * ldr + nx + pc2, ldr); });
            if (rc) break;
            count_gemm(st, o, n, aw, pc);
            doneL = ev.get();
            hipEventRecord(doneL, S);
            hipStreamWaitEvent(S, evB, 0);
            rc = ev.timed(st.ms_gemm, S, [&] { return launch_dgemm_minus(c, ce - cm, n, pc, R + k * ldr + cm, ldr, LT, pc, R + nx * ldr + cm, ldr); });
            if (rc) break;
            count_gemm(st, o, n, ce - cm, pc);
            prevR = doneR;
            doneR = ev.get();
            hipEventRecord(doneR, S);
            chain_a = e2; chain_b = nullptr;
            was_two = true;
            if (o.verbose) printf("panel k=%lld rows=%lld cols=%d (look-ahead, row-major copy, two lanes split at %lld)\n", (long long)nx, (long long)(N - nx), pc2, (long long)cm);
            continue;
        }
        if (was_two) {
            stream_join(ev, T, S);
            if (chain_a) hipStreamWaitEvent(S, chain_a, 0);
            if (chain_b) hipStreamWaitEvent(S, chain_b, 0);
            was_two = false;
        }
        hipEvent_t lt_ready = ev.get();
        {
            stream_join(ev, S, P);
            StreamSwap sw(c, P);
            rc = ev.timed(st.ms_cvt, P, [&] { return launch_transpose64(c, Ap + pc, lda, LT, pc, n, pc, true); });
            hipEventRecord(lt_ready, P);
        }
        if (!rc) rc = ev.timed(st.ms_laswp, S, [&] { return launch_laswp_from_list_rm64(c, R + nx, ldr, ce - nx, lk); });
        if (!rc) rc = ev.timed(st.ms_trsm, S, [&] { return launch_dtrsm_llnu_strided(c, pc, ns, Ap, lda, R + k * ldr + nx, ldr, 1); });
        hipStreamWaitEvent(S, lt_ready, 0);
        if (!rc) rc = ev.timed(st.ms_gemm, S, [&] { return launch_dgemm_minus(c, ns, n, pc, R + k * ldr + nx, ldr, LT, pc, R + nx * ldr + nx, ldr); });
        if (rc) break;
        count_gemm(st, o, n, ns, pc);
        if (!has_next) {
            rc = ev.timed(st.ms_cvt, S, [&] {
                int e = launch_transpose64(c, d_A + nx * lda + k, lda, R + k * ldr + nx, ldr, pc, N - nx, false);
                if (!e) e = launch_transpose64(c, d_A + nx * lda + nx, lda, R + nx * ldr + nx, ldr, N - nx, N - nx, false);
                return e; });
            break;
        }
        rc = ev.timed(st.ms_cvt, S, [&] { return launch_transpose64(c, d_A + nx * lda + nx, lda, R + nx * ldr + nx, ldr, N - nx, pc2, false); });
        if (rc) break;
        hipEvent_t e1 = ev.get();
        hipEventRecord(e1, S);
        const ChainEnd next = chain_behind(f, nx, e1);
        rc = next.rc;
        if (rc) break;
        if (cw > 0) {
            rc = ev.timed(st.ms_trsm, S, [&] { return launch_dtrsm_llnu_strided(c, pc, cw, Ap, lda, R + k * ldr + nx + pc2, ldr, 1); });
            if (rc) break;
        }
        if (T) {
            stream_join(ev, S, T);
            StreamSwap sw(c, T);
            rc = ev.timed(st.ms_cvt, T, [&] { return launch_transpose64(c, d_A + nx * lda + k, lda, R + k * ldr + nx, ldr, pc, ce - nx, false); });
            if (sink && !rc && ce == N) sink_notify(c, (int)(k / nb) + 1, T);
        } else {
            rc = ev.timed(st.ms_cvt, S, [&] { return launch_transpose64(c, d_A + nx * lda + k, lda, R + k * ldr + nx, ldr, pc, ce - nx, false); });
            if (sink && !rc && ce == N) sink_notify(c, (int)(k / nb) + 1, S);
        }
        if (rc) break;
        if (cw > 0) {
            rc = ev.timed(st.ms_gemm, S, [&] { return launch_dgemm_minus(c, cw, n, pc, R + k * ldr + nx + pc2, ldr, LT, pc, R + nx * ldr + nx + pc2, ldr); });
            if (rc) break;
            count_gemm(st, o, n, cw, pc);
        }
        chain_a = next.a; chain_b = next.b;
        hipStreamWaitEvent(S, chain_a, 0);
        if (chain_b) hipStreamWaitEvent(S, chain_b, 0);
        if (o.verbose) printf("panel k=%lld rows=%lld cols=%d (look-ahead, row-major copy)\n", (long long)nx, (long long)(N - nx), pc2);
    }
    if (!rc && lp && lseg < lp->nseg) rc = fail(c, -1, "factor_lookahead_rm: a late column segment was never brought up to date (plan beyond the matrix)");
    if (T) stream_join(ev, T, S);
    stream_join(ev, P, S);
    return factor_epilogue(f, rc, sink, 1, true);
}

static int factor_superpanel(mpf_ctx *c, double *d_A, int64_t lda, int64_t N, int32_t nb, int32_t *d_ipiv, const mpf_opts &o,
                             mpf_stats &st, int sb, bool overlap) {
    hipStream_t S = c->stream, P = overlap ? c->pstream : c->stream;
    hipStream_t Ci = (overlap && c->tstream) ? c->tstream : c->stream;
    const bool lanes = Ci != S;
    EvPool ev(c);
    ev.keep = &st.ms_gemm;
    const FactorArgs f{c, ev, st, o, d_A, lda, N, nb, d_ipiv};
    int rc = 0;
    const bool split = o.trailing == MPF_TRAIL_FP16X3;
    const bool f64 = o.trailing == MPF_TRAIL_FP64;
    const bool use32 = !f64 && c->tune.fp16_work32 != 0 && N > (int64_t)(sb + 1) * nb;
    float *W = nullptr;
    const int64_t ldw = N;
    if (use32) {
        MPF_HIP_TRY(c, c->w32.grow(N * N));
        W = c->w32;
    }
    if (overlap) stream_join(ev, S, P);
    const int64_t sbw = (int64_t)sb * nb;
    const int kst = (int)((sbw + 63) & ~(int64_t)63);
    const int64_t far_cap = N - (int64_t)(sb + 1) * nb;
    const int64_t inner_u_off = (!f64 && far_cap > 0) ? far_cap * kst : 0;
    const int64_t brow_l_off = (int64_t)N * c->h_kmax;
    auto width = [&](int64_t k) { return (int)((N - k) < nb ? (N - k) : nb); };
    auto side_chain = [&](int64_t kx, hipEvent_t e1, hipEvent_t &e2) -> int {
        if (!overlap) return panel_chain(f, kx, S);
        const ChainEnd next = chain_behind(f, kx, e1);
        e2 = next.a;
        if (!next.rc && next.b) {
            e2 = ev.get();
            hipStreamWaitEvent(c->tstream, next.a, 0);
            hipEventRecord(e2, c->tstream);
        }
        return next.rc;
    };
    hipEvent_t img_ready = nullptr;
    auto l21_image = [&](int64_t k, int pc) -> int {
        if (f64) return 0;
        const int64_t mrows = N - k - pc;
        if (mrows <= 0) return 0;
        hipStream_t Is = (lanes && P != S) ? P : Ci;
        if (Is != Ci) stream_join(ev, Ci, Is);
        StreamSwap sw(c, Is);
        int e = ev.timed(st.ms_cvt, Is, [&] { return launch_cvt_l21(c, d_A + k * lda + k + pc, lda, mrows, pc, split); });
        if (Is != Ci) { img_ready = ev.get(); hipEventRecord(img_ready, Is); } else img_ready = nullptr;
        return e;
    };
    auto inner_step = [&](int64_t k, int pc, int64_t col0, int64_t ncols, bool first) -> int {
        if (ncols <= 0) return 0;
        StreamSwap sw(c, Ci);
        double *Ap = d_A + k * lda + k, *A12 = d_A + col0 * lda + k;
        const int64_t mrows = N - k - pc;
        int e = ev.timed(st.ms_trsm, Ci, [&] { return launch_dtrsm_llnu(c, pc, ncols, Ap, lda, A12, lda); });
        if (e || mrows <= 0) return e;
        if (f64) e = ev.timed(st.ms_gemm, Ci, [&] { return launch_dgemm_minus(c, mrows, ncols, pc, Ap + pc, lda, A12, lda, A12 + pc, lda); });
        else {
            e = ev.timed(st.ms_cvt, Ci, [&] { return launch_cvt_u12(c, A12, lda, pc, ncols, split, inner_u_off); });
            if (first && img_ready) hipStreamWaitEvent(Ci, img_ready, 0);
            if (!e) e = ev.timed(st.ms_gemm, Ci, [&] { return launch_hgemm_images(c, mrows, ncols, pc, A12 + pc, lda, false, split, 0, 0, inner_u_off); });
        }
        count_gemm(st, o, mrows, ncols, pc);
        return e;
    };
    struct Far { bool on = false; int64_t s0 = 0, s1 = 0, f0 = 0; int done = 0, img = 1; } far;
    std::vector<hipEvent_t> panel_done;
    auto far_task = [&](int p) -> int {
        const int64_t kq = far.s0 + (int64_t)p * nb, f0 = far.f0, ncols = N - f0;
        if (ncols <= 0) return 0;
        if (lanes) hipStreamWaitEvent(S, panel_done[(size_t)p], 0);
        int e = ev.timed(st.ms_laswp, S, [&] {
            return use32 ? launch_laswp_from_list_f32(c, W + f0, ldw, ncols, c->lists + (kq / nb))
                         : launch_laswp_from_list(c, d_A + f0 * lda, lda, ncols, c->lists + (kq / nb)); });
        if (!e && p > 0) {
            const int K = p * nb;
            if (f64) e = ev.timed(st.ms_trsm, S, [&] {
                return launch_dgemm_minus(c, nb, ncols, K, d_A + far.s0 * lda + kq, lda, d_A + f0 * lda + far.s0, lda, d_A + f0 * lda + kq, lda); }, &st.ms_blockrow);
            else {
                e = ev.timed(st.ms_cvt, S, [&] { return launch_cvt_l21(c, d_A + far.s0 * lda + kq, lda, nb, K, split, 0, brow_l_off); });
                if (!e) e = ev.timed(st.ms_trsm, S, [&] {
                    return use32 ? launch_hgemm_images_rowmajor(c, nb, ncols, K, W + kq * ldw + f0, ldw, split, 0, brow_l_off, 0, 0, kst)
                                 : launch_hgemm_images(c, nb, ncols, K, d_A + f0 * lda + kq, lda, false, split, 0, brow_l_off, 0, 0, kst); }, &st.ms_blockrow);
            }
        }
        if (!e && use32) e = ev.timed(st.ms_cvt, S, [&] { return launch_cvt_f32_f64(c, W + kq * ldw + f0, ldw, d_A + f0 * lda + kq, lda, nb, ncols); });
        if (!e) e = ev.timed(st.ms_trsm, S, [&] { return launch_dtrsm_llnu(c, nb, ncols, d_A + kq * lda + kq, lda, d_A + f0 * lda + kq, lda); }, &st.ms_blockrow);
        if (!e && !f64) e = ev.timed(st.ms_cvt, S, [&] { return launch_cvt_u12(c, d_A + f0 * lda + kq, lda, nb, ncols, split, (int64_t)p * nb, kst); });
        return e;
    };
    auto far_tasks_upto = [&](int ready) -> int {
        int e = 0;
        while (far.on && !e && far.done < ready) { e = far_task(far.done); far.done++; }
        return e;
    };
    auto big_update = [&](const Far &fj, int64_t col0, int64_t ncols) -> int {
        const int64_t mrows = N - fj.s1;
        const int K = (int)(fj.s1 - fj.s0);
        if (ncols <= 0 || mrows <= 0) return 0;
        int e;
        if (f64) e = ev.timed(st.ms_gemm, S, [&] { return launch_dgemm_minus(c, mrows, ncols, K, d_A + fj.s0 * lda + fj.s1, lda, d_A + col0 * lda + fj.s0, lda, d_A + col0 * lda + fj.s1, lda); }, &st.ms_gemm_big);
        else e = ev.timed(st.ms_gemm, S, [&] {
                const int64_t uo = (col0 - fj.f0) * kst;
                return use32 ? launch_hgemm_images_rowmajor(c, mrows, ncols, K, W + fj.s1 * ldw + col0, ldw, split, fj.img, 0, uo, 0, kst)
                             : launch_hgemm_images(c, mrows, ncols, K, d_A + col0 * lda + fj.s1, lda, false, split, fj.img, 0, uo, 0, kst); }, &st.ms_gemm_big);
        const double cb = f64 ? 16.0 : (use32 ? 8.0 : 16.0), opb = f64 ? 8.0 : (split ? 4.0 : 2.0);
        count_gemm(st, o, mrows, ncols, K, cb);
        st.gemm_big_flops += 2.0 * (double)mrows * (double)ncols * K;
        st.gemm_big_bytes += cb * (double)mrows * (double)ncols + opb * K * (double)(mrows + ncols);
        st.gemm_big_launches++;
        return e;
    };
    auto back_to_f64 = [&](int64_t r0, int64_t col0, int64_t ncols) -> int {
        if (!use32 || ncols <= 0) return 0;
        return ev.timed(st.ms_cvt, S, [&] { return launch_cvt_f32_f64(c, W + r0 * ldw + col0, ldw, d_A + col0 * lda + r0, lda, N - r0, ncols); });
    };
    auto inner_end = [&](int64_t c1) { return (c1 + nb) < N ? (c1 + nb) : N; };
    {
        const int64_t e1 = inner_end(sbw < N ? sbw : N);
        if (use32 && e1 < N) rc = ev.timed(st.ms_cvt, S, [&] { return launch_cvt_f64_f32(c, d_A + e1 * lda, lda, W + e1, ldw, N, N - e1); });
    }
    if (!rc) rc = panel_chain(f, 0, S);
    hipEvent_t chain_done = nullptr;
    if (lanes) { chain_done = ev.get(); hipEventRecord(chain_done, S); }
    hipEvent_t ni_ready = nullptr;
    int next_img = 1;
    for (int64_t c0 = 0; c0 < N && rc == 0; c0 += sbw) {
        const int64_t c1 = (c0 + sbw) < N ? (c0 + sbw) : N;
        const int64_t e1c = inner_end(c1);
        const int npan = (int)((c1 - c0 + nb - 1) / nb);
        far = Far();
        if (e1c < N) {
            far.on = true; far.s0 = c0; far.s1 = c1; far.f0 = e1c; far.img = next_img; next_img = 3 - next_img;
            if (!f64 && nb % 64 != 0) {
                const size_t bytes = (size_t)(N - e1c) * kst * sizeof(unsigned short);
// ... 426 lines not shown
```

### mixed-precision_lu_factorization_amd/csrc/mpf_internal.h

```cpp
#pragma once
#include <hip/hip_runtime.h>
#include <stdint.h>
#include <string>
#include <vector>
#include <functional>
#include "../../include/mpf_c.h"

constexpr int HP_R = 256;
constexpr int HP_T = 512;
constexpr int HP_MAXG = 256;
constexpr int HP_MAXCOLS = 256;
constexpr int LASWP_MAXMOVED = 2 * HP_MAXCOLS;

struct MovedList {
    int n;
    int pad[3];
    int src[LASWP_MAXMOVED];
    int dst[LASWP_MAXMOVED];
};

struct MpfWorkspace {
    unsigned long long cand[2][HP_MAXG];
    int flags[16];
    unsigned long long rowbuf[2][HP_MAXG][HP_MAXCOLS / 2];
    int hp_timeouts;
    int pad0[3];
    MovedList list0;
    int info;
    int pad[3];
    unsigned long long hp_stamps[8];
    unsigned long long hp_progress;
    unsigned long long hp_xcd_target;
    unsigned long long hp_xcd_roles;
};

struct MpfTuning {
    int safe_pivots = 0;
    int pivot_fp64 = 0;
    int chain_pipeline = 1;
    long long chain_pipeline_below = 10240;
    int fp16_work32 = 1;
    int superpanel_fp16 = 0;
    int superpanel_fp64 = 1;
    int no_lookahead = 0;
    int verbose = 0;
    int timeline = 0;
    long long hp_spin_limit = 1ll << 21;
    long long hp_gate_ticks = 200000000ll;
    int hp_window = -1;
    int hp_acq_fence = 0;
    int hgemm_pad = 0;
    int hgemm_split_pad = 32768;
    int hgemm_big = 1;
    int hgemm_mfma16 = 1;
    int hgemm_big_tile = 0;
    int dgemm_dma = 1;
    int lazy_gather = 1;
    int dpanel_fused_form = 1;
    int dist_instalments = 1;
    long long dist_instalment_min_bytes = 8ll << 20;
    int generic_fused = 1;
    int fp64_rowmajor = 1;
    long long fp64_rowmajor_min_n = 8192;
    int trsm_laswp_fused = 1;
    int fp64_two_lanes = 8192;
    int dist_solve_p2p = 0;
    int host_sink = 1;
    int hp_local_xcd = 1;
    int hp_half_slabs = 1;
    int hp_half_slabs_rows = 16384;
    int sink_trace = 0;
    int host_late_parts = 3;
    long long host_late_min_n = 16384;
    int host_first_pct = 25;
    int host_late_q_pct = 110;
    long long host_sink_min_n = 4096;
    int gate_wait_value = 0;
    int gesv_fp64_tflops = 0;
    int dist_world1_loop = 0;
    int event_timers = 1;
    int fp64_lane_a_pct = 50;
    int fp64_pair = 1;
    long long fp64_pair_min_n = 16384;
    int gmres_group_tiles = 0;
#ifdef MPF_PROBE
    int hp_stamp = 0;
    int hp_r256_upto = 1 << 30;
    int dgemm_w8 = 1;
    int gemm_lds_pad = 0;
    int hgemm_dbg = 0;
    int hgemm_big_reg = 0;
#endif
};

template <class T, bool Pinned = false>
struct Buf {
    Buf() = default;
    Buf(const Buf &) = delete;
    Buf &operator=(const Buf &) = delete;
    ~Buf() { release(); }
    hipError_t grow(int64_t n) {
        if (n <= cap_) return hipSuccess;
        release();
        void *q = nullptr;
        const hipError_t e = Pinned ? hipHostMalloc(&q, (size_t)n * sizeof(T)) : hipMalloc(&q, (size_t)n * sizeof(T));
        if (e != hipSuccess) return e;
        p_ = (T *)q;
        cap_ = n;
        return hipSuccess;
    }
    void release() {
        if (p_) (void)(Pinned ? hipHostFree(p_) : hipFree(p_));
        p_ = nullptr;
        cap_ = 0;
    }
    T *get() const { return p_; }
    operator T *() const { return p_; }
    int64_t cap() const { return cap_; }
private:
    T *p_ = nullptr;
    int64_t cap_ = 0;
};

struct mpf_ctx {
    MpfTuning tune;
    unsigned attr_done = 0;
    unsigned attr_big = 0;
    int device = 0;
    hipStream_t stream = nullptr;
    bool own_stream = false;
    hipStream_t pstream = nullptr;
    hipStream_t tstream = nullptr;
    hipStream_t xstream = nullptr;
    std::vector<hipEvent_t> ev_pool;
    MpfWorkspace *ws = nullptr;
    hipEvent_t ev0 = nullptr, ev1 = nullptr;
    std::string err;
    mpf_stats stats{};
    int num_cus = 0;
    Buf<double> solve_buf;
    int64_t solve_n = 0;
    Buf<unsigned short> h_L, h_U;
    int64_t h_rows = 0;
    Buf<unsigned short> h_Lb[2];
    int h_kmax = 0;
    unsigned hp_seq = 0;
    unsigned long long *hp_signal = nullptr;
    Buf<int32_t> perm_buf;
    Buf<MovedList> lists;
    Buf<int> Fmap;
    Buf<double> perm_tmp;
    Buf<double> trsv_inv;
    Buf<double> trsv_inv256;
    Buf<int> trsv_cnt;
    Buf<double> krylov;
    Buf<double> res_part;
    Buf<double> ext_part, ext_red, ext_vec;
    Buf<double> blk_tiles, blk_part;
    Buf<int> blk_mask;
    Buf<double> blk_red;
    Buf<int> blk_colarg;
    Buf<double> gm_part, gm_out, gm_ctl;
    Buf<double> dtiles;
    Buf<float> w32;
    Buf<double> r64;
    bool hgemm_standalone = false;
    mpf_p2p_fn p2p_fn = nullptr;
    void *p2p_user = nullptr;
    double gmres_budget_ms = 0;
    double fp64_rate_tflops = 0;
    Buf<double> host_A;
    Buf<int32_t> host_P;
    Buf<double> host_A0;
    Buf<unsigned, true> late_flags;
    unsigned late_seq = 0;
    struct ColFeed *feed = nullptr;
    struct LatePlan *late = nullptr;
    struct RowSink *sink = nullptr;
    Buf<double> rm_tmp;
    Buf<double> rm_lt;
    Buf<double> rm_pair;
    Buf<unsigned short> g16;
    Buf<unsigned long long> gcand;
    Buf<unsigned long long> dpiv;
    Buf<double> dtp;
    void *rccl_comm = nullptr;
    int rccl_rank = 0, rccl_world = 0;
    long long rccl_bcast_calls = 0, rccl_bcast_bytes = 0, rccl_allreduce_calls = 0, rccl_p2p_calls = 0, rccl_p2p_bytes = 0;
    Buf<double> dist_buf[2];
    Buf<float> dist_w32;
    Buf<double> dist_spl;
    int hp_resident_per_cu = -1;
    int hp_win_per_cu = 0;
    int hp_full_beside_waiter = 0;
    int hp_win_beside_waiter = 0;
};

#define MPF_HIP_TRY(ctx, expr)                                                        \
    do {                                                                              \
        hipError_t e_ = (expr);                                                       \
        if (e_ != hipSuccess) {                                                       \
            (ctx)->err = std::string(#expr) + ": " + hipGetErrorString(e_);           \
            return -2;                                                                \
        }                                                                             \
    } while (0)

enum { ATTR_HP = 1, ATTR_DGEMM = 2, ATTR_HGEMM = 4, ATTR_HGEMM256 = 8, ATTR_HGEMM_PP = 16, ATTR_HGEMM16_BIG32 = 32, ATTR_HGEMM16_BIG64 = 64 };
inline bool safe_pivots(const mpf_ctx *c) { return c->tune.safe_pivots != 0; }

int launch_double_to_fp16(mpf_ctx *c, const double *in, uint16_t *out, int64_t n);
int launch_hdiv(mpf_ctx *c, const uint16_t *a, const uint16_t *b, uint16_t *q, int64_t n);
int launch_hgetf2(mpf_ctx *c, const double *A64, int64_t lda, uint16_t *P16, int64_t ld16, int rows,
                  int cols, int ipiv_offset, int *d_ipiv, uint16_t *out16, int64_t ldo, MovedList *moved, int waiters = 0, int prefer_window_rows = 0);
bool hgetf2_lds_eligible(mpf_ctx *c, int rows, int cols);
bool hgetf2_fits_beside(mpf_ctx *c, int rows, int cols, int waiters);
long long hgetf2_capacity_rows(mpf_ctx *c, int waiters, int form = 0);
int laswp_gated_footprint(int *lds_bytes, int *vgprs, int *threads);
int laswp_gated_grid(int64_t ncols);
constexpr int HP_FP64_WINDOW_ROWS = 20000;
int hp_query_residency(mpf_ctx *c);
int launch_hgetf2_gate(mpf_ctx *c, int target);
int launch_laswp_block(mpf_ctx *c, double *A, int64_t lda, int64_t ncols, int k, int cols, const int *d_ipiv, int64_t nrows);
int launch_laswp_block_gated(mpf_ctx *c, double *A, int64_t lda, int64_t ncols, int k, int cols, const int *d_ipiv, int64_t nrows, int target);
int dgetf2_npv_pieces(mpf_ctx *c, int cols);
int launch_dgetf2_npv_piece(mpf_ctx *c, double *P, int64_t ld, int rows, int cols, int fused, int info_base, int piece);
int launch_dpanel_tile_copy(mpf_ctx *c, double *dst, int64_t ld, int piece);
int launch_hgetf2_generic(mpf_ctx *c, const double *A64, int64_t lda, uint16_t *P16, int64_t ld16, int rows, int cols,
                          int ipiv_offset, int *d_ipiv, uint16_t *out16, int64_t ldo);
int launch_laswp_seq(mpf_ctx *c, double *A, int64_t lda, int64_t ncols, int k, int cols, const int *d_ipiv, int64_t nrows);
int launch_laswp_from_list(mpf_ctx *c, double *A, int64_t lda, int64_t ncols, const MovedList *ml);
int launch_laswp_from_list_hole(mpf_ctx *c, double *A, int64_t lda, int64_t ncols, const MovedList *ml, int64_t hole_from, int64_t hole_len);
int launch_lazy_left_swaps(mpf_ctx *c, double *A, int64_t lda, int64_t N, int nb, int npanels, const MovedList *lists, int sb = 1,
                           int world = 1, int rank = 0);
struct LatePlan {
    int nseg = 0;
    int64_t c0[4] = {0, 0, 0, 0};
    int q[4] = {0, 0, 0, 0};
    unsigned *flags = nullptr;
    unsigned seq = 0;
    double *snapshot = nullptr;
    bool taken = false;
    bool snapped[4] = {false, false, false, false};
};
int launch_late_wait(mpf_ctx *c, const unsigned *flag, unsigned seq);
int feed_start(mpf_ctx *c, const double *A_host, double *d_A, int64_t N, LatePlan *lp);
int feed_finish(mpf_ctx *c);
void feed_destroy(mpf_ctx *c);
void feed_trim(mpf_ctx *c);
int sink_attach(mpf_ctx *c, double *A_host, int64_t N, int nb);
bool sink_take(mpf_ctx *c, const double *d_A, int64_t lda, int64_t N, int nb);
void sink_notify(mpf_ctx *c, int upto_panel, hipStream_t stream);
hipError_t sink_stream_wait(mpf_ctx *c, hipStream_t stream);
int sink_finish(mpf_ctx *c, int *panels_sent);
void sink_destroy(mpf_ctx *c);
void sink_trim(mpf_ctx *c);
int launch_laswp(mpf_ctx *c, double *A, int64_t lda, int64_t ncols, int k, int cols, const int *d_ipiv);
int launch_laswp_plan(mpf_ctx *c, const int *d_ipiv, int k, int cols, MovedList *out);
int launch_dgetf2_npv(mpf_ctx *c, double *P, int64_t ld, int rows, int cols, int fused, int info_base);
int launch_dgetf2_piv(mpf_ctx *c, double *P, int64_t ld, int rows, int cols, int fused, int info_base, int ipiv_offset, int *d_ipiv);
int dgetf2_piv_reserve(mpf_ctx *c, int rows);
int launch_dgetf2_tp(mpf_ctx *c, double *P, int64_t ld, int rows, int cols, int fused, int info_base, int ipiv_offset, int *d_ipiv);
int dgetf2_tp_reserve(mpf_ctx *c, int rows);
int launch_dtrsm_llnu(mpf_ctx *c, int m, int64_t n, const double *L, int64_t ldl, double *B, int64_t ldb);
int launch_dgemm_minus(mpf_ctx *c, int64_t m, int64_t n, int k, const double *A, int64_t lda,
                       const double *B, int64_t ldb, double *C, int64_t ldc);
int launch_cvt_l21(mpf_ctx *c, const double *A, int64_t lda, int64_t m, int K, int split, int img = 0, int64_t elem_off = 0);
int launch_hgemm_minus(mpf_ctx *c, int64_t m, int64_t n, int K, const double *B, int64_t ldb, double *C, int64_t ldc,
                       int split, int img = 0, int64_t elem_off = 0);
int launch_hgemm_minus_w32(mpf_ctx *c, int64_t m, int64_t n, int K, const double *B, int64_t ldb, float *C, int64_t ldc,
                           int split, int img = 0, int64_t elem_off = 0);
int launch_cvt_u12(mpf_ctx *c, const double *B, int64_t ldb, int K, int64_t n, int split, int64_t elem_off = 0, int kstride = 0);
int launch_hgemm_images(mpf_ctx *c, int64_t m, int64_t n, int K, void *C, int64_t ldc, bool c32, int split, int img = 0, int64_t elem_off = 0,
                        int64_t u_off = 0, int ksL = 0, int ksU = 0);
struct HgemmImages { const unsigned short *Lh = nullptr, *Ll = nullptr, *Uh = nullptr, *Ul = nullptr; int ksL = 0, ksU = 0; };
int launch_hgemm_ptrs(mpf_ctx *c, int64_t m, int64_t n, int K, const HgemmImages &im, void *C, int64_t ldc, bool c32, int split);
int launch_hgemm16_big(mpf_ctx *c, int64_t m, int64_t n, int Kp, const HgemmImages &im, void *C, int64_t ldc, bool c32);
int launch_hgemm16_ring(mpf_ctx *c, int64_t m, int64_t n, int Kp, const HgemmImages &im, void *C, int64_t ldc, bool c32);
int launch_hgemm_pp(mpf_ctx *c, int64_t m, int64_t n, int Kp, const HgemmImages &im, float *C, int64_t ldc);
int launch_hgemm_images_rowmajor(mpf_ctx *c, int64_t m, int64_t n, int K, float *Crm, int64_t ldrow, int split, int img = 0, int64_t elem_off = 0,
                                 int64_t u_off = 0, int ksL = 0, int ksU = 0);
int launch_laswp_from_list_f32(mpf_ctx *c, float *A, int64_t lda, int64_t ncols, const MovedList *ml);
int launch_laswp_from_list_rm64(mpf_ctx *c, double *R, int64_t ldr, int64_t ncols, const MovedList *ml, int64_t scratch_off = 0);
int launch_transpose64(mpf_ctx *c, double *A, int64_t lda, double *R, int64_t ldr, int64_t rows, int64_t cols, bool to_rowmajor);
int launch_dtrsm_llnu_strided(mpf_ctx *c, int m, int64_t n, const double *L, int64_t ldl, double *B, int64_t rs, int64_t cs);
int launch_cvt_f64_f32(mpf_ctx *c, const double *A, int64_t lda, float *W, int64_t ldw, int64_t rows, int64_t cols);
int launch_cvt_f32_f64(mpf_ctx *c, const float *W, int64_t ldw, double *A, int64_t lda, int64_t rows, int64_t cols);
int launch_gather_rows(mpf_ctx *c, const double *in, const int *perm, double *out, int64_t n);
int launch_residual(mpf_ctx *c, const double *A, int64_t lda, const double *x, const double *b, double *r,
                    int64_t n);
int launch_residual_rect(mpf_ctx *c, const double *A, int64_t lda, const double *x, const double *b, double *r, int64_t n, int64_t ncols);
int launch_trsv_prepare_cols(mpf_ctx *c, const double *LUb, int64_t ld, int64_t n, int64_t k0, int w);
int launch_trsv_lower_cols(mpf_ctx *c, const double *LUb, int64_t ld, double *x, int64_t n, int64_t k0, int w);
int launch_trsv_upper_cols(mpf_ctx *c, const double *LUb, int64_t ld, double *x, int64_t n, int64_t k0, int w);
extern "C" {
int mpf_ensure_h_images(mpf_ctx *c, int64_t rows, int kmax, bool big);
int mpf_ensure_solve_buf(mpf_ctx *c, int64_t n);
int mpf_ensure_rowmajor_copy(mpf_ctx *c, int64_t rows, int64_t cols, int32_t nb);
int mpf_factor_setup(mpf_ctx *c, int64_t N, int32_t nb, int32_t npanels, bool lists);
}
int launch_trsv_prepare(mpf_ctx *c, const double *LU, int64_t ld, int64_t n);
int launch_trsv_lower_unit(mpf_ctx *c, const double *LU, int64_t ld, double *x, int64_t n);
int launch_trsv_upper(mpf_ctx *c, const double *LU, int64_t ld, double *x, int64_t n);
int launch_axpy(mpf_ctx *c, double alpha, const double *x, double *y, int64_t n);
int launch_norm2(mpf_ctx *c, const double *x, int64_t n, double *d_out);
int launch_dot(mpf_ctx *c, const double *x, const double *y, int64_t n, double *d_out);
int launch_scal(mpf_ctx *c, double alpha, double *x, int64_t n);
int solve_setup(mpf_ctx *c, const double *d_LU, int64_t ldlu, const int32_t *d_ipiv, int64_t N);
int solve_check_waits(mpf_ctx *c);
int launch_trsv_upper_t(mpf_ctx *c, const double *LU, int64_t ld, double *x, int64_t n);
int launch_trsv_lower_unit_t(mpf_ctx *c, const double *LU, int64_t ld, double *x, int64_t n);
int launch_scatter_rows(mpf_ctx *c, const double *in, const int *perm, double *out, int64_t n);
int launch_residual_t(mpf_ctx *c, const double *A, int64_t lda, const double *x, const double *b, double *r, int64_t n);
int launch_col_abs_sums(mpf_ctx *c, const double *A, int64_t lda, int64_t m, int64_t n, double *out);
int launch_col_sumsq(mpf_ctx *c, const double *A, int64_t lda, int64_t m, int64_t n, double *out);
int launch_col_max_abs(mpf_ctx *c, const double *A, int64_t lda, int64_t m, int64_t n, const double *rs, double *out);
int launch_row_abs_sums(mpf_ctx *c, const double *A, int64_t lda, int64_t m, int64_t n, double *out);
int launch_row_max_abs(mpf_ctx *c, const double *A, int64_t lda, int64_t m, int64_t n, double *out);
int launch_vec_sum(mpf_ctx *c, const double *x, int64_t n, double *d_out);
int launch_vec_max(mpf_ctx *c, const double *x, int64_t n, double *d_out);
int launch_dasum(mpf_ctx *c, const double *x, int64_t n, double *d_out);
int launch_lacn2_sign(mpf_ctx *c, const double *x, const double *isgn, int64_t n, double *xs, double *d_out);
int launch_idamax(mpf_ctx *c, const double *x, int64_t n, double *d_out);
int launch_lacn2_fill(mpf_ctx *c, double *x, int64_t n, int kind, int64_t j);
int launch_diag_zero(mpf_ctx *c, const double *LU, int64_t ld, int64_t n, double *d_out);
int launch_pow2_scale(mpf_ctx *c, const double *m, int64_t n, double *s, double *d_stats);
int launch_scaled_copy(mpf_ctx *c, const double *A, int64_t lda, const double *r, const double *cs, double *W, int64_t ldw, int64_t m, int64_t n);
int launch_vscale(mpf_ctx *c, const double *x, const double *s, double alpha, double *y, int64_t n);
constexpr int BLK_T = 32;
int launch_blk_tri(mpf_ctx *c, const double *LU, int64_t ld, int64_t n, int which, double *x, double *y, int64_t ldt, int ntiles);
int launch_blk_residual(mpf_ctx *c, const double *A, int64_t lda, int64_t n, bool trans, const double *X, const double *B, double *R,
                        int64_t ldt, int ntiles);
int launch_blk_load(mpf_ctx *c, const double *src, int64_t lds, const int *perm, int64_t n, int64_t ncols, double *t, int64_t ldt, int ntiles,
                    const double *scale = nullptr);
int launch_blk_store(mpf_ctx *c, const double *t, int64_t ldt, const int *perm, int64_t n, int64_t ncols, double *dst, int64_t ldd,
                     const double *scale = nullptr);
int launch_blk_masked_axpy(mpf_ctx *c, const double *d, const int *mask, double *x, int64_t ldt, int ntiles);
int launch_blk_residual_bound(mpf_ctx *c, const double *A, int64_t lda, int64_t n, bool trans, const double *X, const double *B, double *R,
                              double *W, double *Q, int64_t ldt, int ntiles, double safe1, double safe2);
int launch_blk_col_reduce(mpf_ctx *c, int what, const double *T, int64_t ldt, int64_t n, int64_t ncols, const double *sg, const int *at);
int launch_blk_scale(mpf_ctx *c, double *v, const double *w, int64_t ldt, int ntiles);
int launch_blk_ferr_weight(mpf_ctx *c, const double *r, double *w, int64_t n, int64_t ncols, int64_t ldt, double nzeps, double safe1, double safe2);
int launch_blk_lacn2_fill(mpf_ctx *c, double *v, int64_t n, int64_t ncols, int64_t ldt, const int *kind, const int *at);
int launch_blk_lacn2_sign(mpf_ctx *c, double *v, double *isgn, int64_t n, int64_t ncols, int64_t ldt, const int *live);
int blk_refine_core(mpf_ctx *c, bool trans, const double *d_A, int64_t lda, const double *d_LU, int64_t ldlu, int64_t N, int32_t nrhs,
                    const double *d_B, int64_t ldb, double *d_X, int64_t ldx, int32_t max_iter, double tol, const double *pre,
                    const double *post, mpf_ir_stats *st);
int blk_bounds_core(mpf_ctx *c, bool trans, const double *d_A, int64_t lda, const double *d_LU, int64_t ldlu, int64_t N, int32_t nrhs,
                    const double *d_B, int64_t ldb, double *d_X, int64_t ldx, int32_t itmax, double *ferr, double *berr, const double *pre,
                    const double *post, mpf_gerfs_stats *st);
int gmres_ortho_chunks(int64_t ldt);
int launch_gmres_ortho(mpf_ctx *c, const double *V, int64_t vs, int ns, double *W, int64_t ldt, int64_t n, int ntiles, const int *live,
                       double *part, double *out);
int launch_gmres_append(mpf_ctx *c, const double *src, const double *scale, double *dst, int64_t ldt, int64_t n, int ntiles);
int launch_gmres_xupdate(mpf_ctx *c, const double *V, int64_t vs, const double *y, const int *cnt, double *X, int64_t ldt, int64_t n,
                         int ntiles);
int blk_gmres_core(mpf_ctx *c, bool trans, const double *d_A, int64_t lda, const double *d_LU, int64_t ldlu, int64_t N, int32_t nrhs,
                   const double *d_B, int64_t ldb, double *d_X, int64_t ldx, int32_t max_outer, int32_t restart, double tol,
                   mpf_gmres_stats *st);

struct StreamSwap {
    mpf_ctx *c; hipStream_t saved;
    StreamSwap(mpf_ctx *c_, hipStream_t s) : c(c_), saved(c_->stream) { c->stream = s; }
    ~StreamSwap() { c->stream = saved; }
};
struct EvPool {
    mpf_ctx *c; size_t next = 0;
    struct Pair { hipEvent_t a, b; double *acc, *acc2; };
    std::vector<Pair> pairs;
    const double *keep = nullptr;
    explicit EvPool(mpf_ctx *c_) : c(c_) {}
    hipEvent_t get() {
        if (next == c->ev_pool.size()) { hipEvent_t e; hipEventCreate(&e); c->ev_pool.push_back(e); }
        return c->ev_pool[next++];
    }
    int timed(double &acc, hipStream_t s, const std::function<int()> &fn, double *also = nullptr) {
        const int lvl = c->tune.timeline ? 2 : c->tune.event_timers;
        if (lvl == 0 || (lvl == 1 && &acc != keep)) return fn();
        hipEvent_t a = get(), b = get();
        hipEventRecord(a, s);
        int rc = fn();
        hipEventRecord(b, s);
        pairs.push_back({a, b, &acc, also});
        return rc;
    }
    void collect() {
        for (auto &p : pairs) { float ms = 0; if (hipEventElapsedTime(&ms, p.a, p.b) == hipSuccess) { *p.acc += ms; if (p.acc2) *p.acc2 += ms; } }
        if (!pairs.empty() && c->tune.timeline) {
            const double *base = pairs[0].acc;
            for (auto &p : pairs) if (p.acc < base) base = p.acc;
            for (auto &p : pairs) {
                float t0 = 0, t1 = 0;
                hipEventElapsedTime(&t0, pairs[0].a, p.a);
                hipEventElapsedTime(&t1, pairs[0].a, p.b);
                fprintf(stderr, "TL %d %.4f %.4f\n", (int)(p.acc - base), t0, t1);
            }
        }
    }
};

inline void count_gemm(mpf_stats &st, const mpf_opts &o, int64_t m, int64_t n, int64_t k, double c_bytes = 16.0) {
    if (m <= 0 || n <= 0 || k <= 0) return;
    st.gemm_flops += 2.0 * (double)m * (double)n * (double)k;
    const double opb = o.trailing == MPF_TRAIL_FP64 ? 8.0 : (o.trailing == MPF_TRAIL_FP16X3 ? 4.0 : 2.0);
    st.gemm_bytes += c_bytes * (double)m * (double)n + opb * (double)k * (double)(m + n);
    st.gemm_launches++;
}
```

### mixed-precision_lu_factorization_amd/csrc/trailing_f64.hip

```cpp
#include "mpf_internal.h"

typedef double d4_t __attribute__((ext_vector_type(4)));
typedef double d2_t __attribute__((ext_vector_type(2)));
typedef unsigned u2_t __attribute__((ext_vector_type(2)));

__device__ __forceinline__ double buf_load_f64(__amdgpu_buffer_rsrc_t rsrc, unsigned voff, unsigned soff) {
    const u2_t v = __builtin_amdgcn_raw_buffer_load_b64(rsrc, (int)voff, (int)soff, 0);
    return __builtin_bit_cast(double, v);
}
__device__ __forceinline__ __amdgpu_buffer_rsrc_t make_rsrc(const void *p) {
    return __builtin_amdgcn_make_buffer_rsrc(const_cast<void *>(p), 0, 0x7FFFFFFF, 0x00020000);
}

constexpr int GT = 128;
constexpr int GBK = 16;
constexpr int GSA = 144;
constexpr int GSB = GBK + 2;
constexpr int G_LDS_DOUBLES = 2 * GBK * GSA + 2 * GT * GSB;
#ifndef DMA_NEG_BLGP
#define DMA_NEG_BLGP 2
#endif


template <bool EDGE, int NT>
__device__ __forceinline__ void dgemm_tile(long long m, long long n, int K, const double *__restrict__ A, long long lda,
                                           const double *__restrict__ B, long long ldb, double *__restrict__ C,
                                           long long ldc, long long m0, long long n0, double *As, double *Bs) {
    constexpr int THREADS = 64 * 2 * (GT / (16 * NT));
    constexpr int EPT = GBK * GT / THREADS;
    constexpr int KSTEP = THREADS / GT;
    constexpr int NSTEP = THREADS / GBK;
    const int tid = threadIdx.x, lane = tid & 63, wave = tid >> 6;
    const int wm = wave & 1, wn = wave >> 1;
    const int lj = lane & 15, lk = lane >> 4;
    const int mrem = (int)((m - m0) < GT ? (m - m0) : GT), nrem = (int)((n - n0) < GT ? (n - n0) : GT);

    char *Cb = (char *)(C + m0 + n0 * ldc);
    const int crow = wm * 64 + lj, ccol = wn * 16 * NT + lk;
    const unsigned ldc8 = (unsigned)ldc * 8u;
    d4_t acc[NT][4];
#pragma unroll
    for (int nt = 0; nt < NT; ++nt)
#pragma unroll
        for (int rr = 0; rr < 4; ++rr) {
            const int col = ccol + nt * 16 + 4 * rr;
            const unsigned coff = (unsigned)col * ldc8 + (unsigned)crow * 8u;
#pragma unroll
            for (int mt = 0; mt < 4; ++mt) {
                if (!EDGE || (crow + mt * 16 < mrem && col < nrem))
                    acc[nt][mt][rr] = __builtin_nontemporal_load((const double *)(Cb + coff + mt * 128));
                else
                    acc[nt][mt][rr] = 0.0;
            }
        }

    const int mA = tid & (GT - 1), kA0 = tid / GT;
    const int kB = tid & (GBK - 1), nB0 = tid / GBK;
    const unsigned lda8 = (unsigned)lda * 8u, ldb8 = (unsigned)ldb * 8u;
    const unsigned offA0 = (unsigned)mA * 8u + (unsigned)kA0 * lda8;
    const unsigned offB0 = (unsigned)kB * 8u + (unsigned)nB0 * ldb8;
    double ra[EPT], rb[EPT];
    const __amdgpu_buffer_rsrc_t rA = make_rsrc(A + m0), rB = make_rsrc(B + n0 * ldb);
    auto gload = [&](int k0) {
#pragma unroll
        for (int i = 0; i < EPT; ++i) {
            if (!EDGE || (mA < mrem && k0 + kA0 + KSTEP * i < K)) ra[i] = buf_load_f64(rA, offA0, (unsigned)(k0 + KSTEP * i) * lda8);
            else ra[i] = 0.0;
            if (!EDGE || (nB0 + NSTEP * i < nrem && k0 + kB < K)) rb[i] = buf_load_f64(rB, offB0, (unsigned)k0 * 8u + (unsigned)(NSTEP * i) * ldb8);
            else rb[i] = 0.0;
        }
    };
    auto sstore = [&](int buf) {
        double *as = As + buf * GBK * GSA + kA0 * GSA + mA;
        double *bs = Bs + buf * GT * GSB + nB0 * GSB + kB;
#pragma unroll
        for (int i = 0; i < EPT; ++i) {
            as[KSTEP * i * GSA] = -ra[i];
            bs[NSTEP * i * GSB] = rb[i];
        }
    };

    const int nK = (K + GBK - 1) / GBK;
    gload(0);
    sstore(0);
    __syncthreads();
#pragma unroll
    for (int nt = 0; nt < NT; ++nt)
#pragma unroll
        for (int mt = 0; mt < 4; ++mt) asm volatile("" : "+v"(acc[nt][mt]));
    for (int it = 0; it < nK; ++it) {
        const int buf = it & 1;
        if (it + 1 < nK) gload((it + 1) * GBK);
        const double *as = As + buf * GBK * GSA + wm * 64 + lj;
        const double *bs = Bs + buf * GT * GSB + (wn * 16 * NT + lj) * GSB;
#pragma unroll
        for (int kk = 0; kk < GBK; kk += 4) {
            double af[NT], bf[4];
#pragma unroll
            for (int nt = 0; nt < NT; ++nt) af[nt] = bs[nt * 16 * GSB + kk + lk];
#pragma unroll
            for (int mt = 0; mt < 4; ++mt) bf[mt] = as[(kk + lk) * GSA + mt * 16];
#pragma unroll
            for (int nt = 0; nt < NT; ++nt)
#pragma unroll
                for (int mt = 0; mt < 4; ++mt)
                    acc[nt][mt] = __builtin_amdgcn_mfma_f64_16x16x4f64(af[nt], bf[mt], acc[nt][mt], 0, 0, 0);
        }
        if (it + 1 < nK) sstore(buf ^ 1);
        __syncthreads();
    }

#pragma unroll
    for (int nt = 0; nt < NT; ++nt)
#pragma unroll
        for (int rr = 0; rr < 4; ++rr) {
            const int col = ccol + nt * 16 + 4 * rr;
            const unsigned coff = (unsigned)col * ldc8 + (unsigned)crow * 8u;
#pragma unroll
            for (int mt = 0; mt < 4; ++mt)
                if (!EDGE || (crow + mt * 16 < mrem && col < nrem)) __builtin_nontemporal_store(acc[nt][mt][rr], (double *)(Cb + coff + mt * 128));
        }
}

__device__ __forceinline__ void dgemm_tile_of_block(int tiles_m, int tiles_n, int &tm, int &tn) {
    const int nwg = tiles_m * tiles_n;
    const int bid = blockIdx.x;
    const int xcd = bid & 7, q = nwg >> 3, r = nwg & 7;
    const int lin = (xcd < r ? xcd * (q + 1) : r * (q + 1) + (xcd - r) * q) + (bid >> 3);
    const int grp = lin / (tiles_m * 8);
    const int gw = (tiles_n - grp * 8) < 8 ? (tiles_n - grp * 8) : 8;
    const int idx = lin - grp * tiles_m * 8;
    tm = idx / gw; tn = grp * 8 + idx % gw;
}

template <int NT>
__device__ __forceinline__ void dgemm_body(long long m, long long n, int K, const double *__restrict__ A, long long lda,
                                           const double *__restrict__ B, long long ldb, double *__restrict__ C, long long ldc,
                                           int tiles_m, int tiles_n) {
    extern __shared__ __attribute__((aligned(16))) double g_lds[];
    double *As = g_lds;
    double *Bs = g_lds + 2 * GBK * GSA;
    int tm, tn;
    dgemm_tile_of_block(tiles_m, tiles_n, tm, tn);
    const long long m0 = (long long)tm * GT, n0 = (long long)tn * GT;
    const bool edge = (m0 + GT > m) || (n0 + GT > n) || (K % GBK != 0);
    if (edge) dgemm_tile<true, NT>(m, n, K, A, lda, B, ldb, C, ldc, m0, n0, As, Bs);
    else dgemm_tile<false, NT>(m, n, K, A, lda, B, ldb, C, ldc, m0, n0, As, Bs);
}

__global__ __launch_bounds__(256, 2) void dgemm_minus_kernel(long long m, long long n, int K, const double *__restrict__ A,
                                                             long long lda, const double *__restrict__ B, long long ldb,
                                                             double *__restrict__ C, long long ldc, int tiles_m,
                                                             int tiles_n) {
    dgemm_body<4>(m, n, K, A, lda, B, ldb, C, ldc, tiles_m, tiles_n);
}
// ... 26 lines not shown
    extern __shared__ __attribute__((aligned(16))) double g_lds[];
    int tm, tn;
    dgemm_tile_of_block(tiles_m, tiles_n, tm, tn);
    const long long m0 = (long long)tm * GT, n0 = (long long)tn * GT;
    const int tid = threadIdx.x, lane = tid & 63, wave = __builtin_amdgcn_readfirstlane(tid >> 6);
    const int wm = wave & 1, wn = wave >> 1;
    const int lj = lane & 15, lk = lane >> 4;

    char *Cb = (char *)(C + m0 + n0 * ldc);
    const int crow = wm * 64 + 2 * lj, ccol = wn * 32 + lk;
    const unsigned ldc8 = (unsigned)ldc * 8u;
    d4_t acc[2][4];
#pragma unroll
    for (int nt = 0; nt < 2; ++nt)
#pragma unroll
        for (int rr = 0; rr < 4; ++rr) {
            const unsigned coff = (unsigned)(ccol + nt * 16 + 4 * rr) * ldc8 + (unsigned)crow * 8u;
#pragma unroll
            for (int mp = 0; mp < 2; ++mp) {
                const d2_t v = __builtin_nontemporal_load((const d2_t *)(Cb + coff + mp * 256));
                acc[nt][2 * mp][rr] = v[0];
                acc[nt][2 * mp + 1][rr] = v[1];
            }
        }

    constexpr int AI = BK / 8;
    constexpr int BCOLS = 64 / Cfg::CH;
    constexpr int BI = GT / BCOLS / 8;
    const double *ga[AI], *gb[BI];
#pragma unroll
    for (int i = 0; i < AI; ++i) ga[i] = A + m0 + (long long)(wave * AI + i) * lda + lane * 2;
#pragma unroll
    for (int i = 0; i < BI; ++i) {
        const int col = (wave * BI + i) * BCOLS + lane / Cfg::CH, p = lane % Cfg::CH;
        const int q = p ^ ((col >> Cfg::SW_SHIFT) & (Cfg::CH - 1));
        gb[i] = B + (n0 + col) * ldb + q * 2;
    }
    auto issue = [&](int s) {
        double *st = g_lds + (s % NS) * Cfg::STAGE_DBL;
        const long long k0 = (long long)s * BK;
#pragma unroll
        for (int i = 0; i < AI; ++i)
            __builtin_amdgcn_global_load_lds((const __attribute__((address_space(1))) void *)(ga[i] + k0 * lda),
                                             (__attribute__((address_space(3))) void *)(st + (wave * AI + i) * Cfg::DSA), 16, 0, 0);
#pragma unroll
        for (int i = 0; i < BI; ++i)
            __builtin_amdgcn_global_load_lds((const __attribute__((address_space(1))) void *)(gb[i] + k0),
                                             (__attribute__((address_space(3))) void *)(st + Cfg::A_DBL + (wave * BI + i) * BCOLS * BK), 16, 0, 0);
    };
    constexpr int LPS = AI + BI;

    int boff[2], bsw[2];
#pragma unroll
    for (int nt = 0; nt < 2; ++nt) {
        const int nn = wn * 32 + nt * 16 + lj;
        boff[nt] = nn * BK;
        bsw[nt] = (nn >> Cfg::SW_SHIFT) & (Cfg::CH - 1);
    }
    const int nst = K / BK;
    for (int s = 0; s < NS - 1 && s < nst; ++s) issue(s);
    for (int i = 0; i < nst; ++i) {
        if (i + NS - 2 < nst) asm volatile("s_waitcnt vmcnt(%0)" ::"n"((NS - 2) * LPS) : "memory");
        else asm volatile("s_waitcnt vmcnt(0)" ::: "memory");
        __syncthreads();
        if (i + NS - 1 < nst) issue(i + NS - 1);
        const double *as = g_lds + (i % NS) * Cfg::STAGE_DBL + wm * 64 + 2 * lj;
        const double *bs = as - (wm * 64 + 2 * lj) + Cfg::A_DBL;
#pragma unroll
        for (int kk = 0; kk < BK; kk += 4 * RUN) {
            double af[RUN][2], bf[RUN][4];
#pragma unroll
            for (int r = 0; r < RUN; ++r) {
                const int k = kk + 4 * r + lk;
#pragma unroll
                for (int nt = 0; nt < 2; ++nt) af[r][nt] = bs[boff[nt] + (((k >> 1) ^ bsw[nt]) << 1) + (k & 1)];
#pragma unroll
                for (int mp = 0; mp < 2; ++mp) {
                    const d2_t v = *(const d2_t *)(as + k * Cfg::DSA + mp * 32);
                    bf[r][2 * mp] = v[0];
                    bf[r][2 * mp + 1] = v[1];
                }
            }
#pragma unroll
            for (int nt = 0; nt < 2; ++nt)
#pragma unroll
                for (int mt = 0; mt < 4; ++mt)
#pragma unroll
                    for (int r = 0; r < RUN; ++r)
                        acc[nt][mt] = __builtin_amdgcn_mfma_f64_16x16x4f64(af[r][nt], bf[r][mt], acc[nt][mt], 0, 0, DMA_NEG_BLGP);
        }
    }

#pragma unroll
    for (int nt = 0; nt < 2; ++nt)
#pragma unroll
        for (int rr = 0; rr < 4; ++rr) {
            const unsigned coff = (unsigned)(ccol + nt * 16 + 4 * rr) * ldc8 + (unsigned)crow * 8u;
#pragma unroll
            for (int mp = 0; mp < 2; ++mp) {
                const d2_t v = {acc[nt][2 * mp][rr], acc[nt][2 * mp + 1][rr]};
                __builtin_nontemporal_store(v, (d2_t *)(Cb + coff + mp * 256));
            }
        }
}

int launch_dgemm_minus(mpf_ctx *c, int64_t m, int64_t n, int k, const double *A, int64_t lda, const double *B,
                       int64_t ldb, double *C, int64_t ldc) {
    if (m <= 0 || n <= 0 || k <= 0) return 0;
    if (((m + GT - 1) / GT) * ((n + GT - 1) / GT) > 0x7FFFFFFFll) { c->err = "dgemm: too many tiles"; return -1; }
    if (lda > (1ll << 27) || ldb > (1ll << 20) || ldc > (1ll << 20)) { c->err = "dgemm: leading dimension too large for 32-bit tile offsets"; return -1; }
    size_t lds = G_LDS_DOUBLES * sizeof(double);
#ifdef MPF_PROBE
    const int w8 = c->tune.dgemm_w8;
    lds += (size_t)c->tune.gemm_lds_pad;
#else
    const int w8 = 1;
#endif
    const int dma = c->tune.dgemm_dma;
    if (!(c->attr_done & ATTR_DGEMM)) {
        MPF_HIP_TRY(c, hipFuncSetAttribute((const void *)dgemm_minus_kernel8d<16, 2, 1>, hipFuncAttributeMaxDynamicSharedMemorySize, DmaCfg<16, 2, 1>::LDS_BYTES));
        MPF_HIP_TRY(c, hipFuncSetAttribute((const void *)dgemm_minus_kernel, hipFuncAttributeMaxDynamicSharedMemorySize, (int)lds));
        MPF_HIP_TRY(c, hipFuncSetAttribute((const void *)dgemm_minus_kernel8, hipFuncAttributeMaxDynamicSharedMemorySize, (int)lds));
        c->attr_done |= ATTR_DGEMM;
    }
    long long kmax = ((1ll << 31) - 1) / (lda * 8) - GBK;
    const long long kmax_b = ((1ll << 31) - 1 - 128 * ldb * 8) / 8 - GBK;
    if (kmax_b < kmax) kmax = kmax_b;
    kmax = kmax / GBK * GBK;
    if (kmax < GBK) { c->err = "dgemm: leading dimension too large for 32-bit tile offsets"; return -1; }
    auto four = [&](int64_t mm, int64_t nn, int kc, const double *a, const double *b, double *cc) {
        const long long tm = (mm + GT - 1) / GT, tn = (nn + GT - 1) / GT;
        dgemm_minus_kernel<<<(int)(tm * tn), 256, lds, c->stream>>>(mm, nn, kc, a, lda, b, ldb, cc, ldc, (int)tm, (int)tn);
    };
    const int64_t mi = w8 ? m / GT * GT : 0, ni = w8 ? n / GT * GT : 0;
    for (long long k0 = 0; k0 < k; k0 += kmax) {
        const int kc = (int)((k - k0) < kmax ? (k - k0) : kmax);
        const double *a = A + k0 * lda, *b = B + k0;
        const bool dma_ok = dma && ((uintptr_t)a % 16 == 0) && ((uintptr_t)b % 16 == 0) && lda % 2 == 0 && ldb % 2 == 0;
        if (mi > 0 && ni > 0 && kc % GBK == 0) {
            const int g = (int)((mi / GT) * (ni / GT)), tmi = (int)(mi / GT), tni = (int)(ni / GT);
            if (dma_ok && dma == 1) dgemm_minus_kernel8d<16, 2, 1><<<g, 512, DmaCfg<16, 2, 1>::LDS_BYTES, c->stream>>>(mi, ni, kc, a, lda, b, ldb, C, ldc, tmi, tni);
            else
            dgemm_minus_kernel8<<<(int)((mi / GT) * (ni / GT)), 512, lds, c->stream>>>(mi, ni, kc, a, lda, b, ldb, C, ldc, (int)(mi / GT), (int)(ni / GT));
            if (m > mi) four(m - mi, n, kc, a + mi, b, C + mi);
            if (n > ni) four(mi, n - ni, kc, a, b + ni * ldb, C + ni * ldc);
        } else {
            four(m, n, kc, a, b, C);
        }
    }
    MPF_HIP_TRY(c, hipGetLastError());
    return 0;
}

constexpr int TR_T = 16;
constexpr int TR_MAXT = 16;
#define KEEP16(v)                                                                                                              \
    asm volatile("" : "+v"(v[0]), "+v"(v[1]), "+v"(v[2]), "+v"(v[3]), "+v"(v[4]), "+v"(v[5]), "+v"(v[6]), "+v"(v[7]), "+v"(v[8]), \
                 "+v"(v[9]), "+v"(v[10]), "+v"(v[11]), "+v"(v[12]), "+v"(v[13]), "+v"(v[14]), "+v"(v[15]))

template <int CG>
__global__ __launch_bounds__(256, 2) void dtrsm_llnu_kernel(int m, long long n, const double *__restrict__ L, long long ldl,
                                                                        double *B, long long rs, long long cs) {
    __shared__ __attribute__((aligned(16))) double sh[4 * 4 * 256 + 2 * CG * 64 * 4];
    const int tid = threadIdx.x, lane = tid & 63, w = tid >> 6;
    const int mt = (m + TR_T - 1) / TR_T;
    const int li = lane & 15, lk = lane >> 4;

    long long coff[CG];
    bool cok[CG];
#pragma unroll
    for (int g = 0; g < CG; ++g) {
        const long long col = ((long long)blockIdx.x * CG + g) * 16 + li;
        cok[g] = col < n;
        coff[g] = (cok[g] ? col : 0) * cs;
    }
    d4_t R[4][CG];
#pragma unroll
    for (int g = 0; g < CG; ++g) {
        double v[16];
#pragma unroll
        for (int q = 0; q < 16; ++q) {
            const int row = (w + 4 * (q >> 2)) * TR_T + lk + 4 * (q & 3);
            v[q] = B[(row < m ? row : m - 1) * rs + coff[g]];
        }
        KEEP16(v);
#pragma unroll
        for (int q = 0; q < 16; ++q) {
            const int row = (w + 4 * (q >> 2)) * TR_T + lk + 4 * (q & 3);
            R[q >> 2][g][q & 3] = (row < m) ? v[q] : 0.0;
        }
    }
    auto load_l = [&](int bj, double (&f)[4][4]) {
#pragma unroll
        for (int t = 0; t < 4; ++t)
#pragma unroll
            for (int kk = 0; kk < 4; ++kk) {
                const int bi = w + 4 * t, gi = bi * TR_T + li, gk = bj * TR_T + 4 * kk + lk;
                f[t][kk] = (bi > bj && gi < m) ? L[gi + (long long)gk * ldl] : 0.0;
            }
    };
    double lf[4][4];
    if (mt > 1) load_l(0, lf);
    double *shw = sh + w * 1024;
    {
        double v[16];
#pragma unroll
        for (int q = 0; q < 16; ++q) {
            const int e = lane + 64 * q, tt = e >> 8, j = (e >> 4) & 15, i = e & 15;
            const int gi = (w + 4 * tt) * TR_T + i, gj = (w + 4 * tt) * TR_T + j;
            v[q] = L[(gi < m ? gi : m - 1) + (long long)(gj < m ? gj : m - 1) * ldl];
        }
        KEEP16(v);
#pragma unroll
        for (int q = 0; q < 16; ++q) {
            const int e = lane + 64 * q, tt = e >> 8, j = (e >> 4) & 15, i = e & 15;
            const int gi = (w + 4 * tt) * TR_T + i, gj = (w + 4 * tt) * TR_T + j;
            shw[e] = (i > j && gi < m && gj < m) ? v[q] : 0.0;
        }
    }
    __syncthreads();
    {
        const int tt = lane >> 4, c = lane & 15;
        const double *lt = shw + tt * 256;
        double x[TR_T];
#pragma unroll
        for (int i = 0; i < TR_T; ++i) x[i] = (i == c) ? 1.0 : 0.0;
#pragma unroll
        for (int j = 0; j < TR_T; ++j)
#pragma unroll
            for (int i = j + 1; i < TR_T; ++i) {
                x[i] = __builtin_fma(-lt[j * 16 + i], x[j], x[i]);
                if (i == TR_T - 1) __builtin_amdgcn_sched_barrier(0);
            }
        __syncthreads();
#pragma unroll
        for (int i = 0; i < TR_T; ++i) shw[tt * 256 + c * 16 + i] = x[i];
    }
    __syncthreads();
    d4_t *slot = reinterpret_cast<d4_t *>(sh + 4 * 4 * 256);

#pragma unroll
    for (int bj = 0; bj < TR_MAXT; ++bj) {
        if (bj < mt) {
            const int to = bj >> 2;
            const bool owner = (w == (bj & 3));
            d4_t xg[CG];
            if (owner) {
                double inv[4];
#pragma unroll
                for (int kk = 0; kk < 4; ++kk) inv[kk] = shw[to * 256 + (4 * kk + lk) * 16 + li];
#pragma unroll
                for (int g = 0; g < CG; ++g) {
                    d4_t acc = (d4_t){0.0, 0.0, 0.0, 0.0};
#pragma unroll
                    for (int kk = 0; kk < 4; ++kk) acc = __builtin_amdgcn_mfma_f64_16x16x4f64(inv[kk], R[to][g][kk], acc, 0, 0, 0);
                    xg[g] = acc;
                    R[to][g] = acc;
                }
                if (bj + 1 < mt) {
#pragma unroll
                    for (int g = 0; g < CG; ++g) slot[((bj & 1) * CG + g) * 64 + lane] = xg[g];
                }
            }
            if (bj + 1 < mt) {
                asm volatile("s_waitcnt lgkmcnt(0)" ::: "memory");
                __builtin_amdgcn_s_barrier();
                asm volatile("" ::: "memory");
                if (!owner) {
#pragma unroll
                    for (int g = 0; g < CG; ++g) xg[g] = slot[((bj & 1) * CG + g) * 64 + lane];
                }
#pragma unroll
                for (int t = 0; t < 4; ++t) {
                    if (w + 4 * t > bj) {
#pragma unroll
                        for (int g = 0; g < CG; ++g)
#pragma unroll
                            for (int kk = 0; kk < 4; ++kk)
                                R[t][g] = __builtin_amdgcn_mfma_f64_16x16x4f64(lf[t][kk], xg[g][kk], R[t][g], 0, 0, 1 );
                    }
                }
                if (bj + 2 < mt) load_l(bj + 1, lf);
            }
        }
    }
#pragma unroll
    for (int t = 0; t < 4; ++t)
#pragma unroll
        for (int g = 0; g < CG; ++g)
#pragma unroll
            for (int r = 0; r < 4; ++r) {
                const int row = (w + 4 * t) * TR_T + lk + 4 * r;
                if (cok[g] && row < m) B[row * rs + coff[g]] = R[t][g][r];
            }
}

static void dtrsm_launch(mpf_ctx *c, int m, int64_t n, const double *L, int64_t ldl, double *B, int64_t rs, int64_t cs) {
    if (n <= 12288) dtrsm_llnu_kernel<1><<<(int)((n + 15) / 16), 256, 0, c->stream>>>(m, n, L, ldl, B, rs, cs);
    else dtrsm_llnu_kernel<4><<<(int)((n + 63) / 64), 256, 0, c->stream>>>(m, n, L, ldl, B, rs, cs);
}

int launch_dtrsm_llnu(mpf_ctx *c, int m, int64_t n, const double *L, int64_t ldl, double *B, int64_t ldb) {
    if (m <= 0 || n <= 0) return 0;
    for (int i0 = 0; i0 < m; i0 += TR_T * TR_MAXT) {
        const int mb = (m - i0) < TR_T * TR_MAXT ? (m - i0) : TR_T * TR_MAXT;
        if (i0 > 0) {
            const int rc = launch_dgemm_minus(c, mb, n, i0, L + i0, ldl, B, ldb, B + i0, ldb);
            if (rc) return rc;
        }
        dtrsm_launch(c, mb, n, L + i0 + (long long)i0 * ldl, ldl, B + i0, 1, ldb);
    }
    MPF_HIP_TRY(c, hipGetLastError());
    return 0;
}
int launch_dtrsm_llnu_strided(mpf_ctx *c, int m, int64_t n, const double *L, int64_t ldl, double *B, int64_t rs, int64_t cs) {
    if (m <= 0 || n <= 0) return 0;
    if (m > TR_T * TR_MAXT) { c->err = "dtrsm (strided): at most 256 rows"; return -1; }
    dtrsm_launch(c, m, n, L, ldl, B, rs, cs);
    MPF_HIP_TRY(c, hipGetLastError());
    return 0;
}
```

Baseline: 54750.

## Fuse laswp, TRSM, GEMM and transposes of the lookahead strip into one kernel

New measurement: 54860, median of 6. About the same (+0.2%).

```diff
diff --git a/include/mpf_c.h b/include/mpf_c.h
--- a/include/mpf_c.h
+++ b/include/mpf_c.h
@@ -79,6 +79,9 @@
                    int64_t ldb);
 int mpf_dgemm_minus(mpf_ctx *ctx, int64_t m, int64_t n, int32_t k, const double *d_A, int64_t lda,
                     const double *d_B, int64_t ldb, double *d_C, int64_t ldc);
+
+int mpf_strip_step(mpf_ctx *ctx, double *d_A, int64_t lda, double *d_R, int64_t ldr, int64_t nrows, int32_t k, int32_t pc, int32_t ns,
+                   const int32_t *d_ipiv_global, int32_t fused);
 
 int mpf_hgemm_minus(mpf_ctx *ctx, int64_t m, int64_t n, int32_t k, const double *d_A, int64_t lda,
                     const double *d_B, int64_t ldb, double *d_C, int64_t ldc, int32_t split );
diff --git a/mixed-precision_lu_factorization_amd/__init__.py b/mixed-precision_lu_factorization_amd/__init__.py
--- a/mixed-precision_lu_factorization_amd/__init__.py
+++ b/mixed-precision_lu_factorization_amd/__init__.py
@@ -20,7 +20,7 @@
     "mpf_solve_gmres_ir", "mpf_trim", "mpf_dist_set_p2p",
     "mpf_solve_ir_trans", "mpf_lange", "mpf_geequ", "mpf_gecon", "mpf_gesvx",
     "mpf_getrs", "mpf_solve_ir_block", "mpf_gerfs", "mpf_gesvx_block",
-    "mpf_dgetf2_piv", "mpf_solve_gmres_ir_block", "mpf_dgetf2_tp",
+    "mpf_dgetf2_piv", "mpf_solve_gmres_ir_block", "mpf_dgetf2_tp", "mpf_strip_step",
 ]
 PROBE_ONLY_SYMBOLS = ["mpf_microbench", "mpf_debug_mfma4", "mpf_debug_gate", "mpf_debug_hgemm_again"]
 CXX_SYMBOL_MPF = "_Z3MPFPdiiPi"
@@ -145,6 +145,7 @@
     L.mpf_dgetf2_tp.argtypes = [vp, vp, i64, i32, i32, i32, i32, vp, C.POINTER(i32)]
     L.mpf_dtrsm_llnu.argtypes = [vp, i32, i64, vp, i64, vp, i64]
     L.mpf_dgemm_minus.argtypes = [vp, i64, i64, i32, vp, i64, vp, i64, vp, i64]
+    L.mpf_strip_step.argtypes = [vp, vp, i64, vp, i64, i64, i32, i32, i32, vp, i32]
     L.mpf_hgemm_minus.argtypes = [vp, i64, i64, i32, vp, i64, vp, i64, vp, i64, i32]
     L.mpf_hgemm_minus_f32.argtypes = [vp, i64, i64, i32, vp, i64, vp, i64, vp, i64, i32]
     L.mpf_w32_from_f64.argtypes = [vp, vp, i64, vp, i64, i64, i64]
@@ -530,6 +531,14 @@
         self._check(self.L.mpf_dgemm_minus(self.h, m, n, k, _ptr(A), _colmajor_ld(A), _ptr(B), _colmajor_ld(B),
                                            _ptr(Cm), _colmajor_ld(Cm)), "dgemm")
 
+    def strip_step(self, A, R, k, pc, ns, ipiv_global, fused=True):
+        self._bind()
+        nrows = A.shape[0]
+        assert R.dim() == 2 and R.is_contiguous() and R.shape[0] >= nrows, "strip_step: R is a contiguous row-major matrix"
+        assert A.shape[1] >= k + pc + ns and R.shape[1] >= k + pc + ns, "strip_step: the strip lies outside the matrix"
+        self._check(self.L.mpf_strip_step(self.h, _ptr(A), _colmajor_ld(A), _ptr(R), R.stride(0), nrows, k, pc, ns, _ptr(ipiv_global),
+                                          int(fused)), "strip_step")
+
     def hgemm_minus(self, Cm, A, B, split=False):
         self._bind()
         m, n = Cm.shape
diff --git a/mixed-precision_lu_factorization_amd/csrc/mpf_host.cpp b/mixed-precision_lu_factorization_amd/csrc/mpf_host.cpp
--- a/mixed-precision_lu_factorization_amd/csrc/mpf_host.cpp
+++ b/mixed-precision_lu_factorization_amd/csrc/mpf_host.cpp
@@ -50,6 +50,7 @@
     OPT_I(fp64_lane_a_pct, "MPF_FP64_LANE_A_PCT", 20, 90),
     OPT_I(fp64_pair, "MPF_FP64_PAIR", 0, 1),
     OPT_L(fp64_pair_min_n, "MPF_FP64_PAIR_MIN_N", 0, 1ll << 40),
+    OPT_I(fp64_fused_strip, "MPF_FP64_FUSED_STRIP", 0, 2),
     OPT_I(event_timers, "MPF_EVENT_TIMERS", 0, 2),
     OPT_I(dist_world1_loop, "MPF_DIST_WORLD1_LOOP", 0, 1),
     OPT_I(gesv_fp64_tflops, "MPF_GESV_FP64_TFLOPS", 0, 1000),
@@ -321,6 +322,34 @@
     if (!c) return -1;
     if (m > 0 && n > 0 && k > 0 && (lda < m || ldb < k || ldc < m)) return fail(c, -1, "dgemm: bad leading dimension");
     return launch_dgemm_minus(c, m, n, k, d_A, lda, d_B, ldb, d_C, ldc);
+}
+
+int mpf_strip_step(mpf_ctx *c, double *d_A, int64_t lda, double *d_R, int64_t ldr, int64_t nrows, int32_t k, int32_t pc, int32_t ns,
+                   const int32_t *d_ipiv, int32_t fused) {
+    if (!c || !d_A || !d_R || !d_ipiv) return -1;
+    if (pc < 1 || pc > HP_MAXCOLS) return fail(c, -1, "strip_step: 1 <= pc <= 256");
+    const int64_t nx = (int64_t)k + pc, rows = nrows - nx;
+    if (k < 0 || ns < 1 || rows < 1) return fail(c, -1, "strip_step: need k >= 0, ns >= 1 and rows below the panel");
+    if (lda < nrows || ldr < nx + ns) return fail(c, -1, "strip_step: bad leading dimension");
+    MPF_HIP_TRY(c, hipSetDevice(c->device));
+    MovedList *ml = &c->ws->list0;
+    int rc = launch_laswp_plan(c, d_ipiv, k, pc, ml);
+    if (rc) return rc;
+    if (fused) return launch_strip_step(c, d_A, lda, d_R, ldr, k, pc, ns, rows, ml, fused == 2 ? 2 : 1);
+    const int64_t need_tmp = (int64_t)LASWP_MAXMOVED * ns, need_lt = rows * (int64_t)pc;
+    if (need_tmp > c->rm_tmp.cap() || need_lt > c->rm_lt.cap()) {
+        MPF_HIP_TRY(c, hipStreamSynchronize(c->stream));
+        if (need_tmp > c->rm_tmp.cap()) MPF_HIP_TRY(c, c->rm_tmp.grow(need_tmp));
+        if (need_lt > c->rm_lt.cap()) MPF_HIP_TRY(c, c->rm_lt.grow(need_lt));
+    }
+    double *Ap = d_A + (int64_t)k * lda + k, *LT = c->rm_lt;
+    rc = launch_transpose64(c, Ap + pc, lda, LT, pc, rows, pc, true);
+    if (!rc) rc = launch_laswp_from_list_rm64(c, d_R + nx, ldr, ns, ml);
+    if (!rc) rc = launch_dtrsm_llnu_strided(c, pc, ns, Ap, lda, d_R + k * ldr + nx, ldr, 1);
+    if (!rc) rc = launch_dgemm_minus(c, ns, rows, pc, d_R + k * ldr + nx, ldr, LT, pc, d_R + nx * ldr + nx, ldr);
+    if (!rc) rc = launch_transpose64(c, d_A + nx * lda + nx, lda, d_R + nx * ldr + nx, ldr, rows, ns, false);
+    if (!rc) rc = launch_transpose64(c, d_A + nx * lda + k, lda, d_R + k * ldr + nx, ldr, pc, ns, false);
+    return rc;
 }
 
 int mpf_ensure_h_images(mpf_ctx *c, int64_t rows, int kmax, bool big) {
@@ -1009,10 +1038,15 @@
             rc = ev.timed(st.ms_cvt, P, [&] { return launch_transpose64(c, Ap + pc, lda, LT, pc, n, pc, true); });
             hipEventRecord(lt_ready, P);
         }
-        if (!rc) rc = ev.timed(st.ms_laswp, S, [&] { return launch_laswp_from_list_rm64(c, R + nx, ldr, ce - nx, lk); });
-        if (!rc) rc = ev.timed(st.ms_trsm, S, [&] { return launch_dtrsm_llnu_strided(c, pc, ns, Ap, lda, R + k * ldr + nx, ldr, 1); });
-        hipStreamWaitEvent(S, lt_ready, 0);
-        if (!rc) rc = ev.timed(st.ms_gemm, S, [&] { return launch_dgemm_minus(c, ns, n, pc, R + k * ldr + nx, ldr, LT, pc, R + nx * ldr + nx, ldr); });
+        const bool fuse = c->tune.fp64_fused_strip && has_next;
+        if (fuse) {
+            rc = ev.timed(st.ms_gemm, S, [&] { return launch_strip_step(c, d_A, lda, R, ldr, k, pc, (int)ns, n, lk, c->tune.fp64_fused_strip); });
+        } else {
+            rc = ev.timed(st.ms_laswp, S, [&] { return launch_laswp_from_list_rm64(c, R + nx, ldr, ce - nx, lk); });
+            if (!rc) rc = ev.timed(st.ms_trsm, S, [&] { return launch_dtrsm_llnu_strided(c, pc, ns, Ap, lda, R + k * ldr + nx, ldr, 1); });
+            hipStreamWaitEvent(S, lt_ready, 0);
+            if (!rc) rc = ev.timed(st.ms_gemm, S, [&] { return launch_dgemm_minus(c, ns, n, pc, R + k * ldr + nx, ldr, LT, pc, R + nx * ldr + nx, ldr); });
+        }
         if (rc) break;
         count_gemm(st, o, n, ns, pc);
         if (!has_next) {
@@ -1022,24 +1056,30 @@
                 return e; });
             break;
         }
-        rc = ev.timed(st.ms_cvt, S, [&] { return launch_transpose64(c, d_A + nx * lda + nx, lda, R + nx * ldr + nx, ldr, N - nx, pc2, false); });
+        if (!fuse) rc = ev.timed(st.ms_cvt, S, [&] { return launch_transpose64(c, d_A + nx * lda + nx, lda, R + nx * ldr + nx, ldr, N - nx, pc2, false); });
         if (rc) break;
         hipEvent_t e1 = ev.get();
         hipEventRecord(e1, S);
         const ChainEnd next = chain_behind(f, nx, e1);
         rc = next.rc;
         if (rc) break;
+        if (fuse && cw > 0) {
+            rc = ev.timed(st.ms_laswp, S, [&] { return launch_laswp_from_list_rm64(c, R + nx + pc2, ldr, cw, lk); });
+            hipStreamWaitEvent(S, lt_ready, 0);
+            if (rc) break;
+        }
         if (cw > 0) {
             rc = ev.timed(st.ms_trsm, S, [&] { return launch_dtrsm_llnu_strided(c, pc, cw, Ap, lda, R + k * ldr + nx + pc2, ldr, 1); });
             if (rc) break;
         }
+        const int64_t us = fuse ? pc2 : 0;
         if (T) {
             stream_join(ev, S, T);
             StreamSwap sw(c, T);
-            rc = ev.timed(st.ms_cvt, T, [&] { return launch_transpose64(c, d_A + nx * lda + k, lda, R + k * ldr + nx, ldr, pc, ce - nx, false); });
+            rc = ev.timed(st.ms_cvt, T, [&] { return launch_transpose64(c, d_A + (nx + us) * lda + k, lda, R + k * ldr + nx + us, ldr, pc, ce - nx - us, false); });
             if (sink && !rc && ce == N) sink_notify(c, (int)(k / nb) + 1, T);
         } else {
-            rc = ev.timed(st.ms_cvt, S, [&] { return launch_transpose64(c, d_A + nx * lda + k, lda, R + k * ldr + nx, ldr, pc, ce - nx, false); });
+            rc = ev.timed(st.ms_cvt, S, [&] { return launch_transpose64(c, d_A + (nx + us) * lda + k, lda, R + k * ldr + nx + us, ldr, pc, ce - nx - us, false); });
             if (sink && !rc && ce == N) sink_notify(c, (int)(k / nb) + 1, S);
         }
         if (rc) break;
diff --git a/mixed-precision_lu_factorization_amd/csrc/mpf_internal.h b/mixed-precision_lu_factorization_amd/csrc/mpf_internal.h
--- a/mixed-precision_lu_factorization_amd/csrc/mpf_internal.h
+++ b/mixed-precision_lu_factorization_amd/csrc/mpf_internal.h
@@ -81,6 +81,7 @@
     int event_timers = 1;
     int fp64_lane_a_pct = 50;
     int fp64_pair = 1;
+    int fp64_fused_strip = 2;
     long long fp64_pair_min_n = 16384;
     int gmres_group_tiles = 0;
 #ifdef MPF_PROBE
@@ -179,6 +180,7 @@
     struct RowSink *sink = nullptr;
     Buf<double> rm_tmp;
     Buf<double> rm_lt;
+    Buf<double> strip_u;
     Buf<double> rm_pair;
     Buf<unsigned short> g16;
     Buf<unsigned long long> gcand;
@@ -205,7 +207,7 @@
         }                                                                             \
     } while (0)
 
-enum { ATTR_HP = 1, ATTR_DGEMM = 2, ATTR_HGEMM = 4, ATTR_HGEMM256 = 8, ATTR_HGEMM_PP = 16, ATTR_HGEMM16_BIG32 = 32, ATTR_HGEMM16_BIG64 = 64 };
+enum { ATTR_HP = 1, ATTR_DGEMM = 2, ATTR_HGEMM = 4, ATTR_HGEMM256 = 8, ATTR_HGEMM_PP = 16, ATTR_HGEMM16_BIG32 = 32, ATTR_HGEMM16_BIG64 = 64, ATTR_STRIP = 128 };
 inline bool safe_pivots(const mpf_ctx *c) { return c->tune.safe_pivots != 0; }
 
 int launch_double_to_fp16(mpf_ctx *c, const double *in, uint16_t *out, int64_t n);
@@ -283,6 +285,8 @@
 int launch_laswp_from_list_rm64(mpf_ctx *c, double *R, int64_t ldr, int64_t ncols, const MovedList *ml, int64_t scratch_off = 0);
 int launch_transpose64(mpf_ctx *c, double *A, int64_t lda, double *R, int64_t ldr, int64_t rows, int64_t cols, bool to_rowmajor);
 int launch_dtrsm_llnu_strided(mpf_ctx *c, int m, int64_t n, const double *L, int64_t ldl, double *B, int64_t rs, int64_t cs);
+int launch_strip_step(mpf_ctx *c, double *A, int64_t lda, const double *R, int64_t ldr, int64_t k, int pc, int ns, int64_t rows,
+                      const MovedList *ml, int form = 1);
 int launch_cvt_f64_f32(mpf_ctx *c, const double *A, int64_t lda, float *W, int64_t ldw, int64_t rows, int64_t cols);
 int launch_cvt_f32_f64(mpf_ctx *c, const float *W, int64_t ldw, double *A, int64_t lda, int64_t rows, int64_t cols);
 int launch_gather_rows(mpf_ctx *c, const double *in, const int *perm, double *out, int64_t n);
diff --git a/mixed-precision_lu_factorization_amd/csrc/strip_step.hip b/mixed-precision_lu_factorization_amd/csrc/strip_step.hip
--- /dev/null
+++ b/mixed-precision_lu_factorization_amd/csrc/strip_step.hip
@@ -0,0 +1,204 @@
+#include "mpf_internal.h"
+#include "trsm_f64_device.h"
+
+constexpr int SS_CG = 4;
+constexpr int SS_MAXH = 256;
+constexpr int SS_U_DOUBLES = TR_MAXT * SS_CG * 64 * 4;
+constexpr int SS_LDS_BYTES = SS_U_DOUBLES * 8 + (HP_MAXCOLS + SS_MAXH) * 4;
+static_assert(dtrsm_body_lds_doubles<SS_CG>() <= SS_U_DOUBLES, "the TRSM body's LDS lies inside the U image");
+
+struct StripArgs {
+    double *A; long long lda;
+    const double *R; long long ldr;
+    long long k, rows;
+    int pc, ns, h, ncg;
+    const MovedList *ml;
+    double *Ug;
+};
+
+template <bool SOLVE>
+__global__ __launch_bounds__(256) void strip_step_kernel(StripArgs a) {
+    constexpr int CG = SS_CG;
+    extern __shared__ __attribute__((aligned(16))) double ss_lds[];
+    d4_t *U = reinterpret_cast<d4_t *>(ss_lds);
+    int *top_src = reinterpret_cast<int *>(ss_lds + SS_U_DOUBLES);
+    int *row_src = top_src + HP_MAXCOLS;
+    const int tid = threadIdx.x, lane = tid & 63, w = tid >> 6;
+    const int li = lane & 15, lk = lane >> 4;
+    const int cg = (int)(blockIdx.x % (unsigned)a.ncg);
+    const long long rb = blockIdx.x / (unsigned)a.ncg;
+    const long long nx = a.k + a.pc;
+    const long long r0 = rb * a.h;
+    const int col0 = cg * 16 * CG;
+
+    if (SOLVE) for (int i = tid; i < a.pc; i += 256) top_src[i] = (int)(a.k + i);
+    for (int i = tid; i < a.h; i += 256) {
+        const long long r = r0 + i;
+        row_src[i] = (int)(nx + (r < a.rows ? r : a.rows - 1));
+    }
+    __syncthreads();
+    int nm = a.ml->n;
+    if (nm > LASWP_MAXMOVED) nm = LASWP_MAXMOVED;
+    for (int i = tid; i < nm; i += 256) {
+        const long long d = a.ml->dst[i];
+        const int s = a.ml->src[i];
+        if (d >= a.k && d < nx) { if (SOLVE) top_src[d - a.k] = s; }
+        else {
+            const long long q = d - nx - r0;
+            if (q >= 0 && q < a.h && d - nx < a.rows) row_src[q] = s;
+        }
+    }
+    __syncthreads();
+
+    const double *Rs = a.R + nx;
+    int ccol[CG];
+    bool cok[CG];
+#pragma unroll
+    for (int g = 0; g < CG; ++g) {
+        const int col = col0 + g * 16 + li;
+        cok[g] = col < a.ns;
+        ccol[g] = cok[g] ? col : a.ns - 1;
+    }
+    if (!SOLVE) {
+        const d4_t *ug = reinterpret_cast<const d4_t *>(a.Ug) + (long long)cg * (TR_MAXT * CG * 64);
+        for (int i = tid; i < ((a.pc + 15) / 16) * CG * 64; i += 256) U[i] = ug[i];
+    } else {
+        d4_t X[4][CG];
+        dtrsm_llnu_body<CG>(a.pc, a.A + a.k * a.lda + a.k, a.lda, ss_lds,
+                            [&](int row, int g) -> const double * { return Rs + (long long)top_src[row] * a.ldr + ccol[g]; }, X);
+        __syncthreads();
+#pragma unroll
+        for (int t = 0; t < 4; ++t)
+#pragma unroll
+            for (int g = 0; g < CG; ++g) {
+                const int bi = w + 4 * t;
+                d4_t v = X[t][g];
+#pragma unroll
+                for (int r = 0; r < 4; ++r) {
+                    const int row = bi * TR_T + lk + 4 * r;
+                    if (row >= a.pc) v[r] = 0.0;
+                    else if (rb == 0 && cok[g]) a.A[(nx + col0 + g * 16 + li) * a.lda + a.k + row] = v[r];
+                }
+                U[(bi * CG + g) * 64 + lane] = v;
+            }
+    }
+    __syncthreads();
+
+    const int nch = (a.pc + 15) / 16;
+    const double *Lp = a.A + a.k * a.lda + nx;
+    for (int j = 0; j * 64 < a.h; ++j) {
+        const int tl = (w + 4 * j) * 16;
+        if (r0 + tl >= a.rows) break;
+        const long long row = r0 + tl + li;
+        const bool rok = row < a.rows;
+        const double *src = Rs + (long long)row_src[tl + li] * a.ldr;
+        d4_t acc[CG];
+#pragma unroll
+        for (int g = 0; g < CG; ++g)
+#pragma unroll
+            for (int r = 0; r < 4; ++r) {
+                const int col = col0 + g * 16 + lk + 4 * r;
+                acc[g][r] = src[col < a.ns ? col : a.ns - 1];
+            }
+        const double *lp = Lp + (rok ? row : a.rows - 1);
+        auto load_l = [&](int ch, double (&f)[4]) {
+#pragma unroll
+            for (int kk = 0; kk < 4; ++kk) {
+                const int kq = ch * 16 + 4 * kk + lk;
+                const double v = lp[(long long)(kq < a.pc ? kq : a.pc - 1) * a.lda];
+                f[kk] = kq < a.pc ? v : 0.0;
+            }
+        };
+        double l0[4], l1[4] = {0.0, 0.0, 0.0, 0.0}, l2[4] = {0.0, 0.0, 0.0, 0.0};
+        load_l(0, l0);
+        if (nch > 1) load_l(1, l1);
+        for (int ch = 0; ch < nch; ++ch) {
+            if (ch + 2 < nch) load_l(ch + 2, l2);
+#pragma unroll
+            for (int g = 0; g < CG; ++g) {
+                const d4_t u = U[(ch * CG + g) * 64 + lane];
+#pragma unroll
+                for (int kk = 0; kk < 4; ++kk) acc[g] = __builtin_amdgcn_mfma_f64_16x16x4f64(u[kk], l0[kk], acc[g], 0, 0, 2 );
+            }
+#pragma unroll
+            for (int kk = 0; kk < 4; ++kk) { l0[kk] = l1[kk]; l1[kk] = l2[kk]; }
+        }
+        double *dst = a.A + nx + row;
+#pragma unroll
+        for (int g = 0; g < CG; ++g)
+#pragma unroll
+            for (int r = 0; r < 4; ++r) {
+                const int col = col0 + g * 16 + lk + 4 * r;
+                if (rok && col < a.ns) dst[(nx + col) * a.lda] = acc[g][r];
+            }
+    }
+}
+
+__global__ __launch_bounds__(256, 2) void strip_u_kernel(StripArgs a) {
+    __shared__ __attribute__((aligned(16))) double sh[dtrsm_body_lds_doubles<1>()];
+    __shared__ int top_src[HP_MAXCOLS];
+    const int tid = threadIdx.x, lane = tid & 63, w = tid >> 6;
+    const int li = lane & 15, lk = lane >> 4;
+    const long long nx = a.k + a.pc;
+    for (int i = tid; i < a.pc; i += 256) top_src[i] = (int)(a.k + i);
+    __syncthreads();
+    int nm = a.ml->n;
+    if (nm > LASWP_MAXMOVED) nm = LASWP_MAXMOVED;
+    for (int i = tid; i < nm; i += 256) {
+        const long long d = a.ml->dst[i];
+        if (d >= a.k && d < nx) top_src[d - a.k] = a.ml->src[i];
+    }
+    __syncthreads();
+    const int col = (int)blockIdx.x * 16 + li;
+    const bool cok = col < a.ns;
+    const double *Rs = a.R + nx + (cok ? col : a.ns - 1);
+    d4_t X[4][1];
+    dtrsm_llnu_body<1>(a.pc, a.A + a.k * a.lda + a.k, a.lda, sh,
+                       [&](int row, int) -> const double * { return Rs + (long long)top_src[row] * a.ldr; }, X);
+    d4_t *ug = reinterpret_cast<d4_t *>(a.Ug) + (long long)(blockIdx.x / SS_CG) * (TR_MAXT * SS_CG * 64);
+    const int g = (int)(blockIdx.x % SS_CG);
+#pragma unroll
+    for (int t = 0; t < 4; ++t) {
+        const int bi = w + 4 * t;
+        d4_t v = X[t][0];
+#pragma unroll
+        for (int r = 0; r < 4; ++r) {
+            const int row = bi * TR_T + lk + 4 * r;
+            if (row >= a.pc) v[r] = 0.0;
+            else if (cok) a.A[(nx + col) * a.lda + a.k + row] = v[r];
+        }
+        ug[(bi * SS_CG + g) * 64 + lane] = v;
+    }
+}
+
+int launch_strip_step(mpf_ctx *c, double *A, int64_t lda, const double *R, int64_t ldr, int64_t k, int pc, int ns, int64_t rows,
+                      const MovedList *ml, int form) {
+    if (ns <= 0 || rows <= 0) return 0;
+    if (pc < 1 || pc > TR_T * TR_MAXT) { c->err = "strip step: 1 <= panel width <= 256"; return -1; }
+    if (k < 0 || k + pc + rows > 0x7FFFFFFFll) { c->err = "strip step: row index beyond 32 bits"; return -1; }
+    if (!(c->attr_done & ATTR_STRIP)) {
+        MPF_HIP_TRY(c, hipFuncSetAttribute((const void *)strip_step_kernel<true>, hipFuncAttributeMaxDynamicSharedMemorySize, SS_LDS_BYTES));
+        MPF_HIP_TRY(c, hipFuncSetAttribute((const void *)strip_step_kernel<false>, hipFuncAttributeMaxDynamicSharedMemorySize, SS_LDS_BYTES));
+        c->attr_done |= ATTR_STRIP;
+    }
+    const int ncg = (ns + 16 * SS_CG - 1) / (16 * SS_CG);
+    if (form == 2 && c->strip_u.cap() < (int64_t)ncg * SS_U_DOUBLES) {
+        MPF_HIP_TRY(c, hipStreamSynchronize(c->stream));
+        const int64_t most = (int64_t)((HP_MAXCOLS + 16 * SS_CG - 1) / (16 * SS_CG)) * SS_U_DOUBLES;
+        MPF_HIP_TRY(c, c->strip_u.grow((int64_t)ncg * SS_U_DOUBLES > most ? (int64_t)ncg * SS_U_DOUBLES : most));
+    }
+    const int cus = c->num_cus > 0 ? c->num_cus : 256;
+    int h = 64;
+    while (h < SS_MAXH && ((rows + h - 1) / h) * ncg > cus) h *= 2;
+    const int64_t grid = ((rows + h - 1) / h) * ncg;
+    if (grid > 0x7FFFFFFFll) { c->err = "strip step: too many workgroups"; return -1; }
+    const StripArgs a{A, lda, R, ldr, k, rows, pc, ns, h, ncg, ml, form == 2 ? c->strip_u.get() : nullptr};
+    if (form == 2) {
+        strip_u_kernel<<<(ns + 15) / 16, 256, 0, c->stream>>>(a);
+        strip_step_kernel<false><<<(int)grid, 256, SS_LDS_BYTES, c->stream>>>(a);
+    } else {
+        strip_step_kernel<true><<<(int)grid, 256, SS_LDS_BYTES, c->stream>>>(a);
+    }
+    MPF_HIP_TRY(c, hipGetLastError());
+    return 0;
+}
diff --git a/mixed-precision_lu_factorization_amd/csrc/trailing_f64.hip b/mixed-precision_lu_factorization_amd/csrc/trailing_f64.hip
--- a/mixed-precision_lu_factorization_amd/csrc/trailing_f64.hip
+++ b/mixed-precision_lu_factorization_amd/csrc/trailing_f64.hip
@@ -1,6 +1,6 @@
 #include "mpf_internal.h"
-
-typedef double d4_t __attribute__((ext_vector_type(4)));
+#include "trsm_f64_device.h"
+
 typedef double d2_t __attribute__((ext_vector_type(2)));
 typedef unsigned u2_t __attribute__((ext_vector_type(2)));
 
@@ -333,18 +333,11 @@
     return 0;
 }
 
-constexpr int TR_T = 16;
-constexpr int TR_MAXT = 16;
-#define KEEP16(v)                                                                                                              \
-    asm volatile("" : "+v"(v[0]), "+v"(v[1]), "+v"(v[2]), "+v"(v[3]), "+v"(v[4]), "+v"(v[5]), "+v"(v[6]), "+v"(v[7]), "+v"(v[8]), \
-                 "+v"(v[9]), "+v"(v[10]), "+v"(v[11]), "+v"(v[12]), "+v"(v[13]), "+v"(v[14]), "+v"(v[15]))
-
 template <int CG>
 __global__ __launch_bounds__(256, 2) void dtrsm_llnu_kernel(int m, long long n, const double *__restrict__ L, long long ldl,
                                                                         double *B, long long rs, long long cs) {
-    __shared__ __attribute__((aligned(16))) double sh[4 * 4 * 256 + 2 * CG * 64 * 4];
+    __shared__ __attribute__((aligned(16))) double sh[dtrsm_body_lds_doubles<CG>()];
     const int tid = threadIdx.x, lane = tid & 63, w = tid >> 6;
-    const int mt = (m + TR_T - 1) / TR_T;
     const int li = lane & 15, lk = lane >> 4;
 
     long long coff[CG];
@@ -356,115 +349,7 @@
         coff[g] = (cok[g] ? col : 0) * cs;
     }
     d4_t R[4][CG];
-#pragma unroll
-    for (int g = 0; g < CG; ++g) {
-        double v[16];
-#pragma unroll
-        for (int q = 0; q < 16; ++q) {
-            const int row = (w + 4 * (q >> 2)) * TR_T + lk + 4 * (q & 3);
-            v[q] = B[(row < m ? row : m - 1) * rs + coff[g]];
-        }
-        KEEP16(v);
-#pragma unroll
-        for (int q = 0; q < 16; ++q) {
-            const int row = (w + 4 * (q >> 2)) * TR_T + lk + 4 * (q & 3);
-            R[q >> 2][g][q & 3] = (row < m) ? v[q] : 0.0;
-        }
-    }
-    auto load_l = [&](int bj, double (&f)[4][4]) {
-#pragma unroll
-        for (int t = 0; t < 4; ++t)
-#pragma unroll
-            for (int kk = 0; kk < 4; ++kk) {
-                const int bi = w + 4 * t, gi = bi * TR_T + li, gk = bj * TR_T + 4 * kk + lk;
-                f[t][kk] = (bi > bj && gi < m) ? L[gi + (long long)gk * ldl] : 0.0;
-            }
-    };
-    double lf[4][4];
-    if (mt > 1) load_l(0, lf);
-    double *shw = sh + w * 1024;
-    {
-        double v[16];
-#pragma unroll
-        for (int q = 0; q < 16; ++q) {
-            const int e = lane + 64 * q, tt = e >> 8, j = (e >> 4) & 15, i = e & 15;
-            const int gi = (w + 4 * tt) * TR_T + i, gj = (w + 4 * tt) * TR_T + j;
-            v[q] = L[(gi < m ? gi : m - 1) + (long long)(gj < m ? gj : m - 1) * ldl];
-        }
-        KEEP16(v);
-#pragma unroll
-        for (int q = 0; q < 16; ++q) {
-            const int e = lane + 64 * q, tt = e >> 8, j = (e >> 4) & 15, i = e & 15;
-            const int gi = (w + 4 * tt) * TR_T + i, gj = (w + 4 * tt) * TR_T + j;
-            shw[e] = (i > j && gi < m && gj < m) ? v[q] : 0.0;
-        }
-    }
-    __syncthreads();
-    {
-        const int tt = lane >> 4, c = lane & 15;
-        const double *lt = shw + tt * 256;
-        double x[TR_T];
-#pragma unroll
-        for (int i = 0; i < TR_T; ++i) x[i] = (i == c) ? 1.0 : 0.0;
-#pragma unroll
-        for (int j = 0; j < TR_T; ++j)
-#pragma unroll
-            for (int i = j + 1; i < TR_T; ++i) {
-                x[i] = __builtin_fma(-lt[j * 16 + i], x[j], x[i]);
-                if (i == TR_T - 1) __builtin_amdgcn_sched_barrier(0);
-            }
-        __syncthreads();
-#pragma unroll
-        for (int i = 0; i < TR_T; ++i) shw[tt * 256 + c * 16 + i] = x[i];
-    }
-    __syncthreads();
-    d4_t *slot = reinterpret_cast<d4_t *>(sh + 4 * 4 * 256);
-
-#pragma unroll
-    for (int bj = 0; bj < TR_MAXT; ++bj) {
-        if (bj < mt) {
-            const int to = bj >> 2;
-            const bool owner = (w == (bj & 3));
-            d4_t xg[CG];
-            if (owner) {
-                double inv[4];
-#pragma unroll
-                for (int kk = 0; kk < 4; ++kk) inv[kk] = shw[to * 256 + (4 * kk + lk) * 16 + li];
-#pragma unroll
-                for (int g = 0; g < CG; ++g) {
-                    d4_t acc = (d4_t){0.0, 0.0, 0.0, 0.0};
-#pragma unroll
-                    for (int kk = 0; kk < 4; ++kk) acc = __builtin_amdgcn_mfma_f64_16x16x4f64(inv[kk], R[to][g][kk], acc, 0, 0, 0);
-                    xg[g] = acc;
-                    R[to][g] = acc;
-                }
-                if (bj + 1 < mt) {
-#pragma unroll
-                    for (int g = 0; g < CG; ++g) slot[((bj & 1) * CG + g) * 64 + lane] = xg[g];
-                }
-            }
-            if (bj + 1 < mt) {
-                asm volatile("s_waitcnt lgkmcnt(0)" ::: "memory");
-                __builtin_amdgcn_s_barrier();
-                asm volatile("" ::: "memory");
-                if (!owner) {
-#pragma unroll
-                    for (int g = 0; g < CG; ++g) xg[g] = slot[((bj & 1) * CG + g) * 64 + lane];
-                }
-#pragma unroll
-                for (int t = 0; t < 4; ++t) {
-                    if (w + 4 * t > bj) {
-#pragma unroll
-                        for (int g = 0; g < CG; ++g)
-#pragma unroll
-                            for (int kk = 0; kk < 4; ++kk)
-                                R[t][g] = __builtin_amdgcn_mfma_f64_16x16x4f64(lf[t][kk], xg[g][kk], R[t][g], 0, 0, 1 );
-                    }
-                }
-                if (bj + 2 < mt) load_l(bj + 1, lf);
-            }
-        }
-    }
+    dtrsm_llnu_body<CG>(m, L, ldl, sh, [&](int row, int g) -> const double * { return B + row * rs + coff[g]; }, R);
 #pragma unroll
     for (int t = 0; t < 4; ++t)
 #pragma unroll
diff --git a/mixed-precision_lu_factorization_amd/csrc/trsm_f64_device.h b/mixed-precision_lu_factorization_amd/csrc/trsm_f64_device.h
--- /dev/null
+++ b/mixed-precision_lu_factorization_amd/csrc/trsm_f64_device.h
@@ -0,0 +1,130 @@
+#pragma once
+#include "mpf_internal.h"
+
+typedef double d4_t __attribute__((ext_vector_type(4)));
+
+constexpr int TR_T = 16;
+constexpr int TR_MAXT = 16;
+template <int CG>
+constexpr int dtrsm_body_lds_doubles() { return 4 * 4 * 256 + 2 * CG * 64 * 4; }
+
+#define KEEP16(v)                                                                                                              \
+    asm volatile("" : "+v"(v[0]), "+v"(v[1]), "+v"(v[2]), "+v"(v[3]), "+v"(v[4]), "+v"(v[5]), "+v"(v[6]), "+v"(v[7]), "+v"(v[8]), \
+                 "+v"(v[9]), "+v"(v[10]), "+v"(v[11]), "+v"(v[12]), "+v"(v[13]), "+v"(v[14]), "+v"(v[15]))
+
+template <int CG, class RhsAddr>
+__device__ __forceinline__ void dtrsm_llnu_body(int m, const double *__restrict__ L, long long ldl, double *sh, RhsAddr rhs,
+                                                d4_t (&R)[4][CG]) {
+    const int tid = threadIdx.x, lane = tid & 63, w = tid >> 6;
+    const int mt = (m + TR_T - 1) / TR_T;
+    const int li = lane & 15, lk = lane >> 4;
+#pragma unroll
+    for (int g = 0; g < CG; ++g) {
+        double v[16];
+#pragma unroll
+        for (int q = 0; q < 16; ++q) {
+            const int row = (w + 4 * (q >> 2)) * TR_T + lk + 4 * (q & 3);
+            v[q] = *rhs(row < m ? row : m - 1, g);
+        }
+        KEEP16(v);
+#pragma unroll
+        for (int q = 0; q < 16; ++q) {
+            const int row = (w + 4 * (q >> 2)) * TR_T + lk + 4 * (q & 3);
+            R[q >> 2][g][q & 3] = (row < m) ? v[q] : 0.0;
+        }
+    }
+    auto load_l = [&](int bj, double (&f)[4][4]) {
+#pragma unroll
+        for (int t = 0; t < 4; ++t)
+#pragma unroll
+            for (int kk = 0; kk < 4; ++kk) {
+                const int bi = w + 4 * t, gi = bi * TR_T + li, gk = bj * TR_T + 4 * kk + lk;
+                f[t][kk] = (bi > bj && gi < m) ? L[gi + (long long)gk * ldl] : 0.0;
+            }
+    };
+    double lf[4][4];
+    if (mt > 1) load_l(0, lf);
+    double *shw = sh + w * 1024;
+    {
+        double v[16];
+#pragma unroll
+        for (int q = 0; q < 16; ++q) {
+            const int e = lane + 64 * q, tt = e >> 8, j = (e >> 4) & 15, i = e & 15;
+            const int gi = (w + 4 * tt) * TR_T + i, gj = (w + 4 * tt) * TR_T + j;
+            v[q] = L[(gi < m ? gi : m - 1) + (long long)(gj < m ? gj : m - 1) * ldl];
+        }
+        KEEP16(v);
+#pragma unroll
+        for (int q = 0; q < 16; ++q) {
+            const int e = lane + 64 * q, tt = e >> 8, j = (e >> 4) & 15, i = e & 15;
+            const int gi = (w + 4 * tt) * TR_T + i, gj = (w + 4 * tt) * TR_T + j;
+            shw[e] = (i > j && gi < m && gj < m) ? v[q] : 0.0;
+        }
+    }
+    __syncthreads();
+    {
+        const int tt = lane >> 4, c = lane & 15;
+        const double *lt = shw + tt * 256;
+        double x[TR_T];
+#pragma unroll
+        for (int i = 0; i < TR_T; ++i) x[i] = (i == c) ? 1.0 : 0.0;
+#pragma unroll
+        for (int j = 0; j < TR_T; ++j)
+#pragma unroll
+            for (int i = j + 1; i < TR_T; ++i) {
+                x[i] = __builtin_fma(-lt[j * 16 + i], x[j], x[i]);
+                if (i == TR_T - 1) __builtin_amdgcn_sched_barrier(0);
+            }
+        __syncthreads();
+#pragma unroll
+        for (int i = 0; i < TR_T; ++i) shw[tt * 256 + c * 16 + i] = x[i];
+    }
+    __syncthreads();
+    d4_t *slot = reinterpret_cast<d4_t *>(sh + 4 * 4 * 256);
+
+#pragma unroll
+    for (int bj = 0; bj < TR_MAXT; ++bj) {
+        if (bj < mt) {
+            const int to = bj >> 2;
+            const bool owner = (w == (bj & 3));
+            d4_t xg[CG];
+            if (owner) {
+                double inv[4];
+#pragma unroll
+                for (int kk = 0; kk < 4; ++kk) inv[kk] = shw[to * 256 + (4 * kk + lk) * 16 + li];
+#pragma unroll
+                for (int g = 0; g < CG; ++g) {
+                    d4_t acc = (d4_t){0.0, 0.0, 0.0, 0.0};
+#pragma unroll
+                    for (int kk = 0; kk < 4; ++kk) acc = __builtin_amdgcn_mfma_f64_16x16x4f64(inv[kk], R[to][g][kk], acc, 0, 0, 0);
+                    xg[g] = acc;
+                    R[to][g] = acc;
+                }
+                if (bj + 1 < mt) {
+#pragma unroll
+                    for (int g = 0; g < CG; ++g) slot[((bj & 1) * CG + g) * 64 + lane] = xg[g];
+                }
+            }
+            if (bj + 1 < mt) {
+                asm volatile("s_waitcnt lgkmcnt(0)" ::: "memory");
+                __builtin_amdgcn_s_barrier();
+                asm volatile("" ::: "memory");
+                if (!owner) {
+#pragma unroll
+                    for (int g = 0; g < CG; ++g) xg[g] = slot[((bj & 1) * CG + g) * 64 + lane];
+                }
+#pragma unroll
+                for (int t = 0; t < 4; ++t) {
+                    if (w + 4 * t > bj) {
+#pragma unroll
+                        for (int g = 0; g < CG; ++g)
+#pragma unroll
+                            for (int kk = 0; kk < 4; ++kk)
+                                R[t][g] = __builtin_amdgcn_mfma_f64_16x16x4f64(lf[t][kk], xg[g][kk], R[t][g], 0, 0, 1 );
+                    }
+                }
+                if (bj + 2 < mt) load_l(bj + 1, lf);
+            }
+        }
+    }
+}
```
